# Cogito2012/OpenTAL

Hardware: AMD Instinct MI355X
Metric: clips/sec training step, 256-frame THUMOS14 clips (higher is better)
Workload: dtype bf16

## Files before the change

include/opental_hip.h:

```cpp
#ifndef OPENTAL_HIP_H
#define OPENTAL_HIP_H

#include <stdint.h>
#include <stddef.h>

#ifdef __cplusplus
extern "C" {
#endif

#define OTAL_ABI_VERSION 26

#define OTAL_E_NULL      (-1)
#define OTAL_E_SHAPE     (-2)
#define OTAL_E_ODD_C     (-3)
#define OTAL_E_BATCH     (-4)
#define OTAL_E_DTYPE     (-5)
#define OTAL_E_LEVELS    (-6)
#define OTAL_E_UNSUPPORTED (-7)

#define OTAL_F32  0
#define OTAL_BF16 1
#define OTAL_F16  2
#define OTAL_F64  3

#define OTAL_MAX_LEVELS 8

int otal_abi_version(void);
const char* otal_error_string(int code);
int otal_set_option(const char* name, int value);
int otal_get_option(const char* name, int dflt);
int otal_stream_wait(void* waiter, void* signaler);

int otal_bmp_fwd(const void* in, const float* seg, void* out,
                 int B, int C, int T, int N, int seg_batch, int dtype, void* stream);

int otal_bmp_bwd(const void* grad_out, const void* in, const float* seg, void* grad_in,
                 int B, int C, int T, int N, int seg_batch, int compat_ref_stride,
                 int dtype, void* stream);

int otal_bmp_fwd_levels(const void* in, const float* seg, void* out,
                        int B, int C, int nlev, const int* t_start, const int* n_start,
                        int dtype, void* stream);
int otal_bmp_bwd_levels(const void* grad_out, const void* in, const float* seg, void* grad_in,
                        int B, int C, int nlev, const int* t_start, const int* n_start,
                        int dtype, void* stream);

int otal_conv_half_storage(const int* geom, const int64_t* strides, int mode, int precision);
size_t otal_conv_workspace_bytes(const int* geom, int mode);

int otal_conv_fwd(const int* geom, const int64_t* strides, const float* x, const float* w,
                  const float* scale, const float* shift, float* y, int relu, int precision,
                  const void* prologue, void* ws, size_t ws_bytes, void* stream);

int otal_conv_dgrad(const int* geom, const int64_t* strides, const float* dy, const float* wt_packed,
                    float* dx, int accumulate, const float* out_mask, const float* out_scale,
                    int precision, const void* prologue, void* ws, size_t ws_bytes, void* stream);

int otal_conv_wgrad(const int* geom, const int64_t* strides, const float* x, const float* dy,
                    float* dw, int accumulate, int precision, const void* prologue, void* ws, size_t ws_bytes,
                    void* stream);

int otal_conv_fwd_pair(const int* geom, const int64_t* strides, const float* const* x, const float* const* w,
                       const float* const* scale, const float* const* shift, float* const* y, int relu, int precision,
                       const void* const* prologue, void* ws, size_t ws_bytes, void* stream);
int otal_conv_dgrad_pair(const int* geom, const int64_t* strides, const float* const* dy, const float* const* w,
                         float* const* dx, int precision, const void* const* prologue, void* ws, size_t ws_bytes, void* stream);
int otal_conv_wgrad_pair(const int* geom, const int64_t* strides, const float* const* x, const float* const* dy,
                         float* const* dw, int precision, void* ws, size_t ws_bytes, void* stream);

size_t otal_conv_prologue_bytes(const int* geom, const int64_t* strides, int mode, int precision);
size_t otal_conv_prologue_desc_bytes(void);
int otal_conv_prologue(const int* geom, const int64_t* strides, int mode, const float* w, int precision, void* region,
                       size_t region_bytes, void* host_desc, void* stream);
int otal_conv_prologue_batch(int n, const void* device_descs, const int* device_starts, int total_blocks, void* stream);

int otal_conv_defer_reduces(int on);
size_t otal_conv_deferred_end(void);
int otal_conv_deferred_count(void);
int otal_conv_flush_reduces(void* stream);

const char* otal_conv_last_kernel(void);

int otal_conv_pack_wt(const float* w, float* wt, int Cout, int Cin, int kvol, void* stream);

int otal_gn_relu_fwd(const float* x, const float* gamma, const float* beta, float* y, float* stats,
                     int B, int C, int T, int G, float eps, int relu, int nlev, const int* lev, void* stream);
int otal_gn_relu_bwd(const float* dy, int64_t dy_batch_stride, const float* x, const float* gamma, const float* beta,
                     const float* stats, float* dx, float* partial, int B, int C, int T, int G,
                     int relu, int nlev, const int* lev, void* stream);
int otal_gn_relu_fwd_pair(const float* const* x, const float* const* gamma, const float* const* beta, float* const* y,
                          float* const* stats, int B, int C, int T, int G, float eps, int relu, int nlev, const int* lev,
                          void* stream);
int otal_gn_relu_bwd_pair(const float* const* dy, const int64_t* dy_batch_stride, const float* const* x,
                          const float* const* gamma, const float* const* beta, const float* const* stats, float* const* dx,
                          float* const* partial, int B, int C, int T, int G, int relu, int nlev, const int* lev, void* stream);
int otal_sum_partials(int n_items, const float* const* partial, float* const* dst0, float* const* dst1,
                      float* const* dst2, const int* channels, const int* batches, void* stream);

const char* otal_layer_last_kernel(void);

int otal_maxpool3d_fwd(const int* geom, const int64_t* strides, const float* x, float* y,
                       unsigned char* argtap, void* stream);
int otal_maxpool3d_bwd(const int* geom, const int64_t* strides, const float* dy,
                       const unsigned char* argtap, float* dx, int accumulate,
                       const float* out_mask, const float* out_scale, void* stream);
size_t otal_maxpool3d_signbits_bytes(const int* geom, const int64_t* strides);
int otal_maxpool3d_fwd_signbits(const int* geom, const int64_t* strides, const float* x, float* y,
                                unsigned char* argtap, unsigned char* signbits, void* stream);
int otal_maxpool3d_bwd_signbits(const int* geom, const int64_t* strides, const float* dy, const unsigned char* argtap,
                                float* dx, int accumulate, const unsigned char* signbits, const float* out_scale,
                                void* stream);
int otal_maxpool3d_fwd_signbits_h(const int* geom, const int64_t* strides, const void* x_bf16, float* y,
                                  unsigned char* argtap, unsigned char* signbits, void* stream);
int otal_maxpool3d_bwd_signbits_h(const int* geom, const int64_t* strides, const float* dy, const unsigned char* argtap,
                                  void* dx_bf16, const unsigned char* signbits, const float* out_scale, void* stream);
int otal_maxpool3d_fwd_io(const int* geom, const int64_t* strides, const void* x, void* y, unsigned char* argtap,
                          unsigned char* signbits, int io, void* stream);
int otal_maxpool3d_bwd_io(const int* geom, const int64_t* strides, const void* dy, const unsigned char* argtap, void* dx,
                          int accumulate, const void* out_mask, const float* out_scale, const unsigned char* signbits, int io,
                          void* stream);
int otal_convert_storage(const void* src, int64_t src_bs, int64_t src_cs, void* dst, int64_t dst_bs, int64_t dst_cs,
                         int to_bf16, int B, int C, int P, void* stream);

int otal_head_outputs_fwd(int n_items, const int* channels, const int* modes, const float* const* raw, float* const* out,
                          float* const* unct, const float* scales, int B, int N, int nlev, const int* lev,
                          const float* level_strides, void* stream);
int otal_head_outputs_bwd(int n_items, const int* channels, const int* modes, const float* const* raw,
                          const float* const* out, const float* const* unct, const float* const* dout,
                          const float* const* dunct, float* const* draw, const float* scales, float* dscales, int B,
                          int N, int nlev, const int* lev, const float* level_strides, void* stream);

int otal_boundary_bce(const float* x, int64_t x_batch_stride, int64_t x_channel_stride, const float* mask,
                      int64_t mask_batch_stride, int64_t mask_row_stride, int mask_row0, int mask_step, float* terms,
                      float* dx, int B, int C, int T, void* stream);

int otal_boundary_finish(int n, const float* const* terms, const float* weights, const int* T, int B, float* out2, void* stream);
int otal_boundary_scale(int n, const float* const* dx, float* const* out, const float* weights, const int* C, const int* T,
                        int B, const float* g_start, const float* g_end, void* stream);

int otal_proposal_windows(const float* loc, float* seg, float* frame_seg, int B, int nlev,
                          const int* lev, float frame_num, void* stream);

int otal_decode_clips(const float* loc, const float* prop_loc, const float* priors, const float* conf,
                      const float* prop_conf, const float* center, const float* act, const float* prop_act,
                      const float* offsets, const float* fps, float* seg, float* score, float* unct,
                      float* actn, unsigned char* flag, int nclips, int A, int K, float clip_length,
                      float conf_thresh, void* stream);
int otal_decode_clips_ex(const float* loc, const float* prop_loc, const float* priors, const float* conf,
                         const float* prop_conf, const float* center, const float* act, const float* prop_act,
                         const float* offsets, const float* fps, float* seg, float* score, float* unct,
                         float* actn, unsigned char* flag, int nclips, int A, int K, float clip_length,
                         float conf_thresh, int score_fn, int first_class, void* stream);
int otal_decode_clips_ev(const float* loc, const float* prop_loc, const float* priors, const float* conf,
                         const float* prop_conf, const float* center, const float* act, const float* prop_act,
                         const float* offsets, const float* fps, float* seg, float* score, float* unct,
                         float* actn, unsigned char* flag, int nclips, int A, int K, float clip_length,
                         float conf_thresh, int score_fn, int first_class, int evidence, void* stream);
int otal_decode_clips_2s(const float* loc, const float* prop_loc, const float* conf, const float* prop_conf,
                         const float* center, const float* act, const float* prop_act, const float* flow_loc,
                         const float* flow_prop_loc, const float* flow_conf, const float* flow_prop_conf,
                         const float* flow_center, const float* flow_act, const float* flow_prop_act,
                         const float* unct_in, const float* prop_unct_in, const float* flow_unct_in,
                         const float* flow_prop_unct_in, const float* priors, const float* offsets, const float* fps,
                         float* seg, float* score, float* unct, float* actn, unsigned char* flag, int nclips, int A, int K,
                         float clip_length, float conf_thresh, int score_fn, int first_class, int evidence, int conf_sign,
                         void* stream);
int otal_softnms_classes(const float* seg, const float* score, const float* unct, const float* actn,
                         const unsigned char* flag, const int* clip_start, int nvideos, int max_clips,
                         int A, int K, float sigma, int top_k, float score_threshold, float* out,
                         int* counts, int* out_index, int out_cols, void* stream);
size_t otal_softnms_scratch_bytes(int total_clips, int max_clips, int A, int K);
int otal_softnms_classes_ws(const float* seg, const float* score, const float* unct, const float* actn,
                            const unsigned char* flag, const int* clip_start, int nvideos, int max_clips,
                            int A, int K, float sigma, int top_k, float score_threshold, float* out,
                            int* counts, int* out_index, int out_cols, void* scratch, size_t scratch_bytes,
                            int total_clips, void* stream);
int otal_detection_table(const float* rows, const int* counts, const double* durations, int V, int K, int top_k, int cols,
                         int drop_empty, int scoring, int* video, int* cls, double* seg, float* sup, double* known,
                         int* list_start, void* stream);
int otal_anchor_stats(const float* loc, const float* conf, const float* prop_conf, const float* center, const float* act,
                      const float* prop_act, const float* priors, const float* gt, const unsigned char* gvalid, int B, int K,
                      int C, int G, float clip_length, float overlap_thresh, int os_head, int n_known, int target,
                      int score_bins, int grad_bins, long long* hist_score, long long* hist_grad, int* label, float* value,
                      float* grad, void* stream);
int otal_anchor_stats_ev(const float* loc, const float* conf, const float* prop_conf, const float* center, const float* act,
                         const float* prop_act, const float* priors, const float* gt, const unsigned char* gvalid, int B,
                         int K, int C, int G, float clip_length, float overlap_thresh, int os_head, int n_known, int target,
                         int score_bins, int grad_bins, long long* hist_score, long long* hist_grad, int* label,
                         float* value, float* grad, int evidence, void* stream);

int otal_openmax_dist(const float* feat, int N, int rows_per_batch, int64_t sb, int64_t sr, int64_t sc, const float* mav,
                      int K, int D, const int* labels, float* dist, void* stream);
int otal_openmax_class_means(const float* feat, int N, int rows_per_batch, int64_t sb, int64_t sr, int64_t sc,
                             const int* labels, int K, int D, float* means, int* counts, void* stream);
int otal_openmax_probs(const float* logits, int64_t ldl, const float* feat, int N, int rows_per_batch, int64_t sb, int64_t sr,
                       int64_t sc, const float* mav, const float* wb, int K, int D, int R, float* probs, void* stream);
int otal_decode_clips_openmax(const float* loc, const float* prop_loc, const float* priors, const float* conf,
                              const float* prop_conf, const float* center, const float* offsets, const float* fps,
                              const float* feat, const float* prop_feat, const int64_t* feat_strides,
                              const int64_t* prop_feat_strides, const float* mav, const float* mav_prop, const float* wb,
                              const float* wb_prop, float* seg, float* score, float* unknown, unsigned char* flag,
                              int nclips, int A, int C, int first_class, int D, int R, int refined_feature,
                              float clip_length, float conf_thresh, void* stream);

int otal_openmax_dist_wide(const float* feat, int N, int rows_per_batch, int64_t sb, int64_t sr, int64_t sc, const float* mav,
                           int K, int D, const int* labels, float* dist, void* stream);
int otal_openmax_probs_wide(const float* logits, int64_t ldl, const float* feat, int N, int rows_per_batch, int64_t sb,
                            int64_t sr, int64_t sc, const float* mav, const float* wb, int K, int D, int R, float* probs,
                            void* stream);
int otal_decode_clips_openmax_wide(const float* loc, const float* prop_loc, const float* priors, const float* conf,
                                   const float* prop_conf, const float* center, const float* offsets, const float* fps,
                                   const float* feat, const float* prop_feat, const int64_t* feat_strides,
                                   const int64_t* prop_feat_strides, const float* mav, const float* mav_prop, const float* wb,
                                   const float* wb_prop, float* seg, float* score, float* unknown, unsigned char* flag,
                                   int nclips, int A, int C, int first_class, int D, int R, int refined_feature,
                                   float clip_length, float conf_thresh, void* stream);

int otal_head_convs_supported(int n_heads, int n_inputs, const int* in_idx, const int* cout, const int* ksize, int B, int C, int N);
int otal_head_convs_fwd(int n_heads, int n_inputs, const int* in_idx, const int* cout, const int* ksize,
                        const float* const* x, const float* const* w, const float* const* bias, float* const* y, int B, int C,
                        int N, int nlev, const int* lev, void* stream);
int otal_head_convs_bwd(int n_heads, int n_inputs, const int* in_idx, const int* cout, const int* ksize,
                        const float* const* x, const float* const* w, const float* const* dy, float* const* dx,
                        float* const* dw, float* const* db, int B, int C, int N, int nlev, const int* lev, void* stream);
int otal_head_convs_bwd_parts(int n_heads, int n_inputs, const int* in_idx, const int* cout, const int* ksize,
                        const float* const* x, const float* const* w, const float* const* dy, float* const* dx,
                        float* const* dw, float* const* db, int B, int C, int N, int nlev, const int* lev, int parts, void* stream);

int otal_rpl_head_fwd(const float* x, const float* centers, float* dist, int B, int C, int D, int N, void* stream);
int otal_rpl_head_bwd(const float* x, const float* centers, const float* g, float* dx, float* dcenters, int B, int C, int D,
                      int N, int parts, void* stream);

int otal_masked_scale_copy(const float* src, const int64_t* src_strides, const float* z, const int64_t* z_strides,
                           const float* scale, float* dst, const int64_t* dst_strides, int accumulate, int B, int C,
                           int T, int S, void* stream);

int otal_adam_flat(float* p, const float* g, float* m, float* v, int64_t n, float lr, float beta1,
                   float beta2, float eps, float weight_decay, int step, float grad_scale, void* stream);

int otal_adam_flat_dev(float* p, const float* g, float* m, float* v, int64_t n, float lr, float beta1,
                       float beta2, float eps, float weight_decay, const float* bias_corr, float grad_scale,
                       void* stream);

#define OTAL_GRAD_NORM_PARTIALS 2048
int otal_grad_norm(const float* g, int64_t n, float grad_scale, float max_norm, double* partials, float* out, void* stream);

int otal_adam_flat_clip(float* p, const float* g, float* m, float* v, int64_t n, float lr, float beta1, float beta2,
                        float eps, float weight_decay, const float* bias_corr, float grad_scale, const float* norm_coef,
                        void* stream);

size_t otal_detection_loss_scratch_floats(int B, int K);
size_t otal_detection_loss_grad_floats(int B, int K, int C);
int otal_detection_loss(const float* loc, const float* conf, const float* prop_loc, const float* prop_conf,
                        const float* center, const float* act, const float* prop_act, const float* priors,
                        const float* gt, const unsigned char* gvalid, float* weight_accum, int B, int K, int C, int G,
                        float clip_length, float overlap_thresh, int ibm_active, int num_bins, float momentum,
                        int iou_aware, int cls_mode, float focal_alpha, float* losses, float* grads, float* scratch,
                        void* stream);

int otal_detection_loss_ex(const float* loc, const float* conf, const float* prop_loc, const float* prop_conf,
                           const float* center, const float* act, const float* prop_act, const float* priors,
                           const float* gt, const unsigned char* gvalid, float* weight_accum, int B, int K, int C, int G,
                           float clip_length, float overlap_thresh, int ibm_active, int num_bins, float momentum,
                           int iou_aware, int cls_mode, float focal_alpha, int reweight, float rw_gamma, float* losses,
                           float* grads, float* scratch, void* stream);
int otal_detection_loss_ev(const float* loc, const float* conf, const float* prop_loc, const float* prop_conf,
                           const float* center, const float* act, const float* prop_act, const float* priors,
                           const float* gt, const unsigned char* gvalid, float* weight_accum, int B, int K, int C, int G,
                           float clip_length, float overlap_thresh, int ibm_active, int num_bins, float momentum,
                           int iou_aware, int cls_mode, float focal_alpha, int reweight, float rw_gamma, int evidence,
                           int loss_type, float* losses, float* grads, float* scratch, void* stream);

int otal_detection_loss_anet(const float* loc, const float* conf, const float* prop_loc, const float* prop_conf,
                             const float* center, const float* act, const float* prop_act, const float* priors2,
                             const float* gt, const unsigned char* gvalid, int B, int K, int C, int G,
                             float clip_length, float overlap_thresh, const float* level_bounds, int nlev,
                             int ibm_active, float ibm_coeff, int iou_aware, float act_weight, float act_margin,
                             float* losses, float* grads, float* scratch, void* stream);
int otal_detection_loss_anet_ex(const float* loc, const float* conf, const float* prop_loc, const float* prop_conf,
                                const float* center, const float* act, const float* prop_act, const float* priors2,
                                const float* gt, const unsigned char* gvalid, int B, int K, int C, int G,
                                float clip_length, float overlap_thresh, const float* level_bounds, int nlev,
                                int ibm_active, float ibm_coeff, int iou_aware, float act_weight, float act_margin,
                                int cls_mode, float focal_alpha, float* losses, float* grads, float* scratch, void* stream);
int otal_detection_loss_anet_ev(const float* loc, const float* conf, const float* prop_loc, const float* prop_conf,
                                const float* center, const float* act, const float* prop_act, const float* priors2,
                                const float* gt, const unsigned char* gvalid, int B, int K, int C, int G,
                                float clip_length, float overlap_thresh, const float* level_bounds, int nlev,
                                int ibm_active, float ibm_coeff, int iou_aware, float act_weight, float act_margin,
                                int cls_mode, float focal_alpha, int evidence, int loss_type, float* losses, float* grads,
                                float* scratch, void* stream);

int otal_detection_loss_rpl(const float* loc, const float* conf, const float* prop_loc, const float* prop_conf,
                            const float* center, const float* priors, const float* gt, const unsigned char* gvalid,
                            int B, int K, int C, int G, float clip_length, float overlap_thresh, int gcpl,
                            float temperature, float weight_pl, float radius, float* losses, float* grads, float* scratch,
                            void* stream);

int otal_detection_loss_bwd(const float* grads, const float* const* g7, float* out, int B, int K, int C, void* stream);

int otal_prepare_clips(const unsigned char* frames, const void* params, float* out, int B, int T, int Hs, int Ws,
                       int Ho, int Wo, void* stream);
int otal_prepare_clips_map(const unsigned char* frames, const void* params, const int* frame_map, float* out,
                           float* out_ssl, int B, int T, int Hs, int Ws, int Ho, int Wo, void* stream);
int otal_prepare_clips_ch(const unsigned char* frames, const void* params, const int* frame_map, float* out, float* out_ssl,
                          int B, int C_src, int C_out, int T, int Hs, int Ws, int Ho, int Wo, void* stream);

int otal_prepare_windows(const void* params, float* out, int B, int C, int T, int H, int W, void* stream);


int otal_pyramid_merge_fwd(const float* p0, const float* p1, float* packed, float* frame, int B, int C, int t0, int T,
                           int up, void* stream);
int otal_pyramid_merge_bwd(const float* da, const float* db, const float* dframe, const float* dnext, float* dp0, float* dp1,
                           int B, int C, int t0, int T, int up, void* stream);
int otal_gn_relu_fwd_to(const float* x, const float* gamma, const float* beta, float* y, int64_t y_bs, int64_t y_cs,
                        float* stats, int B, int C, int T, int G, float eps, int relu, int nlev, const int* lev, void* stream);
int otal_gn_relu_fwd_pair_to(const float* const* x, const float* const* gamma, const float* const* beta, float* const* y,
                             int64_t y_bs, int64_t y_cs, float* const* stats, int B, int C, int T, int G, float eps, int relu,
                             int nlev, const int* lev, void* stream);

int otal_gn_relu_bwd_sum(int n_terms, const float* const* dy, const int64_t* dy_bs, const int64_t* dy_cs, const int* dy_T,
                         const float* x, const float* gamma, const float* beta, const float* stats, float* dx, float* partial,
                         int B, int C, int T, int G, int relu, int nlev, const int* lev, void* stream);

int otal_bmp_fwd_levels_to(const float* in, const float* seg, float* out, int64_t pooled_bs, int B, int C, int nlev,
                           const int* t_start, const int* n_start, void* stream);
int otal_bmp_bwd_levels_from(const float* grad_out, int64_t pooled_bs, const float* in, const float* seg, float* grad_in, int B,
                             int C, int nlev, const int* t_start, const int* n_start, void* stream);

#define OTAL_EVAL_MAX_GT 1024
int otal_eval_match(const double* pred_seg, const int* pred_start, const double* gt_seg, const int* gt_start,
                    const double* thresholds, int ngroups, int nthr, int* out, int* nonfinite, void* stream);

int otal_eval_match_labeled(const double* pred_seg, const int* pred_label, const int* pred_start, const double* gt_seg,
                            const int* gt_label, const int* gt_start, const double* thresholds, int ngroups, int nthr, int* out,
                            double* max_tiou, int* nonfinite, void* stream);

#define OTAL_AP_TILE 256
#define OTAL_AP_MAX_CLASS_ROWS (2147483647 - OTAL_AP_TILE)
int otal_average_precision(const int* codes, const int* rank_pos, const int* class_start, const int* gt_count, int N, int K,
                           int nthr, double* ap, void* stream);

int otal_open_set_curves(const double* known, const int* flags, int M, int nthr, double* out, void* stream);

#define OTAL_WI_MAX_GT 16777216
int otal_wilderness_impact(const int* codes, const int* pred_label, const int* gt_label, int n_known, int n_unknown, int N,
                           int M, int nthr, int K, double* out, void* stream);

#ifdef __cplusplus
}
#endif
#endif
```

opental_amd/common/i3d_backbone.py:

```python
import torch
import torch.nn as nn
import torch.nn.functional as F
from torch.autograd import Function

from . import ops
from .layers import MaxPool3dSamePadding

ONE, THREE = (1, 1, 1), (3, 3, 3)
BN_EPS = 1e-3


class Unit3D(nn.Module):

    def __init__(self, in_channels, output_channels, kernel_shape=(1, 1, 1), stride=(1, 1, 1), padding=0,
                 activation_fn=F.relu, use_batch_norm=True, use_bias=False, padding_valid_spatial=False,
                 name='unit_3d'):
        super(Unit3D, self).__init__()
        if not use_batch_norm or use_bias or activation_fn is not F.relu or padding_valid_spatial or padding == -1:
            raise NotImplementedError("backbone Unit3D is conv(no bias) + BN + ReLU with SAME padding")
        self._output_channels = output_channels
        self._kernel_shape = tuple(kernel_shape)
        self._stride = tuple(stride)
        self.name = name
        self.conv3d = nn.Conv3d(in_channels, output_channels, self._kernel_shape, self._stride, padding=0, bias=False)
# ... 6 lines not shown

    def forward(self, x):
        scale, shift = self.folded_bn()
        return I3DFeaturesFunction.apply(x, [("conv", 0, self._kernel_shape, self._stride)], ("out",), scale, shift,
                                         [0, scale.numel()], self.conv3d.weight)[0]


class InceptionModule(nn.Module):
    def __init__(self, in_channels, out_channels, name):
        super(InceptionModule, self).__init__()
        oc = out_channels
        self.b0 = Unit3D(in_channels, oc[0], ONE, name=name + '/Branch_0/Conv3d_0a_1x1')
        self.b1a = Unit3D(in_channels, oc[1], ONE, name=name + '/Branch_1/Conv3d_0a_1x1')
        self.b1b = Unit3D(oc[1], oc[2], THREE, name=name + '/Branch_1/Conv3d_0b_3x3')
        self.b2a = Unit3D(in_channels, oc[3], ONE, name=name + '/Branch_2/Conv3d_0a_1x1')
        self.b2b = Unit3D(oc[3], oc[4], THREE, name=name + '/Branch_2/Conv3d_0b_3x3')
        self.b3a = MaxPool3dSamePadding(kernel_size=[3, 3, 3], stride=(1, 1, 1), padding=0)
        self.b3b = Unit3D(in_channels, oc[5], ONE, name=name + '/Branch_3/Conv3d_0b_1x1')
        self.name = name
        self.out_channels = tuple(oc)

    def units(self):
        return [self.b0, self.b1a, self.b1b, self.b2a, self.b2b, self.b3b]

    def fused_1x1_weights(self):
        return [self.b1a.conv3d.weight, self.b2a.conv3d.weight, self.b0.conv3d.weight]


_ENDPOINTS = (
    ('Conv3d_1a_7x7', 'conv', (None, 64, (7, 7, 7), (2, 2, 2))),
    ('MaxPool3d_2a_3x3', 'pool', ((1, 3, 3), (1, 2, 2))),
    ('Conv3d_2b_1x1', 'conv', (64, 64, ONE, ONE)),
    ('Conv3d_2c_3x3', 'conv', (64, 192, THREE, ONE)),
    ('MaxPool3d_3a_3x3', 'pool', ((1, 3, 3), (1, 2, 2))),
    ('Mixed_3b', 'mixed', (192, (64, 96, 128, 16, 32, 32))),
    ('Mixed_3c', 'mixed', (256, (128, 128, 192, 32, 96, 64))),
    ('MaxPool3d_4a_3x3', 'pool', (THREE, (2, 2, 2))),
    ('Mixed_4b', 'mixed', (480, (192, 96, 208, 16, 48, 64))),
    ('Mixed_4c', 'mixed', (512, (160, 112, 224, 24, 64, 64))),
    ('Mixed_4d', 'mixed', (512, (128, 128, 256, 24, 64, 64))),
    ('Mixed_4e', 'mixed', (512, (112, 144, 288, 32, 64, 64))),
    ('Mixed_4f', 'mixed', (528, (256, 160, 320, 32, 128, 128))),
    ('MaxPool3d_5a_2x2', 'pool', ((2, 2, 2), (2, 2, 2))),
    ('Mixed_5b', 'mixed', (832, (256, 160, 320, 32, 128, 128))),
    ('Mixed_5c', 'mixed', (832, (384, 192, 384, 48, 128, 128))),
)


class ExtendWeightFunction(Function):

    @staticmethod
    def forward(ctx, w2, buf):
        if w2.dim() != 5 or w2.shape[1] != 2 or tuple(buf.shape) != (w2.shape[0], 3) + tuple(w2.shape[2:]) \
                or buf.dtype != w2.dtype or buf.device != w2.device:
            raise RuntimeError("ExtendWeightFunction: a (Cout,2,kt,kh,kw) weight and a (Cout,3,kt,kh,kw) buffer of its dtype / device")
        buf[:, :2].copy_(w2.detach())
        ctx.w2 = w2
        return buf.detach()

    @staticmethod
    def backward(ctx, g3):
        w2, ctx.w2 = ctx.w2, None
        slot = ops.grad_slot(w2) if g3.is_cuda else None
        if slot is not None:
            slot.copy_(g3[:, :2])
            return slot, None
        return g3[:, :2].contiguous(), None


def check_clip_planes(weight_channels, x):
    from .input_pipeline import is_zero_plane
    planes = int(x.shape[1])
    if weight_channels == 2 and planes == 3:
        if not is_zero_plane(x):
            raise RuntimeError("a 2-channel (optical-flow) network was handed a 3-plane clip batch that is not flagged as a "
                               "zero-plane flow batch (rgb frames?): flow batches come from ClipStager(channels=2) / "
                               "prepare_clips on (T,H,W,2) frames")
        return True
    if is_zero_plane(x) and weight_channels != 2:
        raise RuntimeError(f"a zero-plane optical-flow batch was handed to a network with {weight_channels} input channels "
                           "(in_channels must be 2)")
    if planes != weight_channels:
        raise RuntimeError(f"clip batch has {planes} planes, the network's first layer takes {weight_channels} "
                           "(rgb clips have 3, optical-flow clips 2)")
    return False


class InceptionI3d(nn.Module):
    VALID_ENDPOINTS = tuple(n for n, _, _ in _ENDPOINTS) + ('Logits', 'Predictions')

    def __init__(self, num_classes=400, spatial_squeeze=True, final_endpoint='Mixed_5c', name='inception_i3d',
                 in_channels=3, dropout_keep_prob=0.5):
        super(InceptionI3d, self).__init__()
        if final_endpoint not in self.VALID_ENDPOINTS:
            raise ValueError('Unknown final endpoint %s' % final_endpoint)
        if final_endpoint in ('Logits', 'Predictions'):
            raise NotImplementedError("the detection path stops at Mixed_5c (BDNet.py:27)")
        self._final_endpoint = final_endpoint
        self.end_points = {}
        for ep, kind, args in _ENDPOINTS:
            if kind == 'conv':
                cin, cout, k, s = args
                self.end_points[ep] = Unit3D(in_channels if cin is None else cin, cout, k, s, name=name + ep)
            elif kind == 'pool':
                self.end_points[ep] = MaxPool3dSamePadding(kernel_size=list(args[0]), stride=args[1], padding=0)
            else:
                self.end_points[ep] = InceptionModule(args[0], list(args[1]), name + ep)
            if ep == final_endpoint:
                break
        self._plan = None

    def build(self):
        for k in self.end_points.keys():
            self.add_module(k, self.end_points[k])

    def _make_plan(self):
        plan, units = [], []
        for ep, kind, args in _ENDPOINTS:
            if ep not in self.end_points:
                break
            mod = self.end_points[ep]
            if kind == 'conv':
                plan.append(("conv", len(units), mod._kernel_shape, mod._stride))
                units.append(mod)
            elif kind == 'pool':
                plan.append(("pool", tuple(mod.kernel_size), tuple(mod.stride)))
            else:
                plan.append(("mixed", len(units), mod.out_channels))
                units += mod.units()
            plan[-1] = plan[-1] + (ep,)
        return plan, units

    def extract_features(self, x, endpoints=('Mixed_4f', 'Mixed_5c')):
        if self._plan is None:
            self._plan = self._make_plan()
        plan, units = self._plan
        zero_plane = check_clip_planes(int(units[0].conv3d.weight.shape[1]), x)
        for u in units:
            if u.bn.training or (torch.is_grad_enabled() and u.bn.weight.requires_grad):
                raise NotImplementedError("I3D BatchNorm must be frozen (freeze_bn + freeze_bn_affine, BDNet.py:39-49)")
        key = tuple((u.bn.weight._version, u.bn.bias._version, u.bn.running_mean._version, u.bn.running_var._version,
                     u.bn.weight.data_ptr(), u.bn.running_var.data_ptr()) for u in units)
        if getattr(self, "_fold_key", None) != key:
            folded = [u.folded_bn() for u in units]
            offs = [0]
            for sc, _ in folded:
                offs.append(offs[-1] + sc.numel())
            self._fold = (torch.cat([sc for sc, _ in folded]), torch.cat([sh for _, sh in folded]), offs)
            self._fold_key = key
        scale, shift, offs = self._fold
        weights = [u.conv3d.weight for u in units]
        if zero_plane:
            weights[0] = ExtendWeightFunction.apply(weights[0], self._extended_weight(weights[0]))
        cut = self._stem_cut(plan, endpoints) if self.split_backward else 0
        if cut:
            (stem_out,) = I3DFeaturesFunction.apply(x, plan[:cut], ("=" + plan[cut - 1][-1],), scale, shift, offs, *weights)
            self.stem_out = cut_in = stem_out
            if self.detach_cut and torch.is_grad_enabled() and stem_out.requires_grad:
                self.cut_leaf = cut_in = stem_out.detach().requires_grad_(True)
            outs = I3DFeaturesFunction.apply(cut_in, plan[cut:], tuple(endpoints), scale, shift, offs, *weights)
        else:
            self.stem_out = None
            outs = I3DFeaturesFunction.apply(x, plan, tuple(endpoints), scale, shift, offs, *weights)
        return dict(zip(endpoints, outs))

    _w3 = None

    def _extended_weight(self, w2):
        buf = self._w3
        if buf is None or buf.device != w2.device or buf.dtype != w2.dtype:
            if w2.is_cuda and torch.cuda.is_current_stream_capturing():
                raise RuntimeError("the zero-plane weight buffer cannot be created inside a graph capture: run one eager "
                                   "forward pass of the flow network first")
            buf = self._w3 = torch.zeros((w2.shape[0], 3) + tuple(w2.shape[2:]), dtype=w2.dtype, device=w2.device)
        return buf

    split_backward = False
    detach_cut = False
    stem_out = None
    cut_leaf = None
    STEM_CUT_AFTER = 'MaxPool3d_4a_3x3'

    def _stem_cut(self, plan, endpoints):
        names = [st[-1] for st in plan]
        if self.STEM_CUT_AFTER not in names:
            return 0
        cut = names.index(self.STEM_CUT_AFTER) + 1
        if cut >= len(plan) or any(e in names[:cut] for e in endpoints):
            return 0
        return cut

    def stem_parameters(self):
        if self._plan is None:
            self._plan = self._make_plan()
        plan, units = self._plan
        cut = self._stem_cut(plan, ())
        idx = set()
        for st in plan[:cut]:
            if st[0] == "conv":
                idx.add(st[1])
            elif st[0] == "mixed":
                idx.update(range(st[1], st[1] + 6))
        return [units[i].conv3d.weight for i in sorted(idx)]

    def forward(self, x):
        raise NotImplementedError("classification logits are not part of the detection path; use extract_features")


_FUSED_AFFINE = {}


def _fused_weight(w_b1a, w_b2a, w_b0):
    n1, n2 = w_b1a.numel(), w_b2a.numel()
    es = w_b1a.element_size()
    if (w_b1a.is_contiguous() and w_b2a.is_contiguous() and w_b0.is_contiguous()
            and w_b2a.data_ptr() == w_b1a.data_ptr() + n1 * es and w_b0.data_ptr() == w_b2a.data_ptr() + n2 * es
            and w_b1a.untyped_storage().data_ptr() == w_b0.untyped_storage().data_ptr()):
        rows = w_b1a.shape[0] + w_b2a.shape[0] + w_b0.shape[0]
        return w_b1a.as_strided((rows,) + tuple(w_b1a.shape[1:]), w_b1a.stride(), w_b1a.storage_offset())
    return torch.cat([w_b1a, w_b2a, w_b0], 0)


def _cat_cached(cache, owner, tag, parts):
    key = (owner.data_ptr(), owner._version, tag)
    hit = cache.get(key)
    if hit is None:
        hit = (torch.cat(parts), owner)
        if len(cache) > 256:
            cache.clear()
        cache[key] = hit
    return hit[0]


_OUT_SCALE = {}


def _fused_affine(scale, shift, offs, w0):
    key = (scale.data_ptr(), shift.data_ptr(), scale._version, w0)
    hit = _FUSED_AFFINE.get(key)
    if hit is None:
        pick = lambda t, i: t[offs[i]:offs[i + 1]]
        hit = (torch.cat([pick(scale, w0 + 1), pick(scale, w0 + 3), pick(scale, w0)]),
               torch.cat([pick(shift, w0 + 1), pick(shift, w0 + 3), pick(shift, w0)]), scale, shift)
        if len(_FUSED_AFFINE) > 256:
            _FUSED_AFFINE.clear()
        _FUSED_AFFINE[key] = hit
    return hit[0], hit[1]


_HALF_OK = {}


def _pool_half_ok(shape, k, s):
    _, _, T, H, W = shape
    k, s = tuple(k), tuple(s)
    out_positions = -(-T // s[0]) * -(-H // s[1]) * -(-W // s[2])
    if out_positions % 8:
        return False
    if k[1:] == (3, 3) and s[1:] == (2, 2) and H % 2 == 0 and W % 4 == 0:
        return (k[0], s[0]) == (1, 1) or ((k[0], s[0]) == (3, 2) and T % 2 == 0)
    return k == THREE and s == ONE and H == W and H in (12, 6)


def _conv_half_ok(shape, cout, k, first=False):
    modes = (0, 2) if first else (0, 1, 2)
    return all(ops.half_storage_ok(m, tuple(shape), cout, k, ONE, both=True) for m in modes)


def _step_half_ok(step, shape, weights):
    key = (step[0], tuple(shape), step[1:-1] if step[0] != "conv" else (tuple(weights[step[1]].shape), step[2], step[3]), ops.HALF_CHAIN,
           int(ops.CONV_PRECISION), ops.HALF_STORAGE)
    hit = _HALF_OK.get(key)
    if hit is None:
        B, C, T, H, W = shape
        if not (ops.HALF_CHAIN and ops.HALF_STORAGE and int(ops.CONV_PRECISION) & 1):
            hit = False
        elif step[0] == "conv":
            hit = tuple(step[3]) == ONE and _conv_half_ok(shape, weights[step[1]].shape[0], tuple(step[2]))
        elif step[0] == "pool":
            hit = _pool_half_ok(shape, step[1], step[2])
        else:
            oc = step[2]
            hit = (_conv_half_ok(shape, oc[1] + oc[3] + oc[0], ONE) and _conv_half_ok((B, oc[1], T, H, W), oc[2], THREE)
                   and _conv_half_ok((B, oc[3], T, H, W), oc[4], THREE) and _pool_half_ok(shape, THREE, ONE)
                   and _conv_half_ok(shape, oc[5], ONE))
        if len(_HALF_OK) > 512:
            _HALF_OK.clear()
        _HALF_OK[key] = hit
    return hit


class I3DFeaturesFunction(Function):

    @staticmethod
    def forward(ctx, x, plan, endpoints, scale, shift, offs, *weights):
        x = x.contiguous()
        sc = lambda i: scale[offs[i]:offs[i + 1]]
        sh = lambda i: shift[offs[i]:offs[i + 1]]
        tape, found, half_grads = [], {}, {}
        cur = x
        cur_scale = None
        BF = torch.bfloat16
        need_grad = any(ctx.needs_input_grad)
        raw_out = {e[1:] for e in endpoints if e.startswith("=")}
        endpoints = tuple(e.lstrip("=") for e in endpoints)

        def leave_half():
            nonlocal cur
            cur32 = ops.convert_storage(cur, torch.float32)
            tape.append(("cvt", cur, cur32, cur_scale))
            cur = cur32

        for si, step in enumerate(plan):
            kind, name = step[0], step[-1]
            chain = cur.dtype == BF and _step_half_ok(step, cur.shape, weights)
            pool_io1 = (cur.dtype == BF and not chain and kind == "pool" and cur_scale is not None
                        and tuple(step[1]) == (1, 3, 3) and tuple(step[2]) == (1, 2, 2)
                        and cur.shape[3] % 2 == 0 and cur.shape[4] % 4 == 0)
            if cur.dtype == BF and not chain and not pool_io1:
                leave_half()
            if kind == "conv" and chain:
                _, wi, k, s, _ = step
                y = ops.conv_forward(cur, weights[wi], k, s, scale=sc(wi), shift=sh(wi), relu=True)
                tape.append(("conv", wi, k, s, cur, y, cur_scale, sc(wi)))
                cur, cur_scale = y, sc(wi)
            elif kind == "conv":
                _, wi, k, s, _ = step
                pooled_next = (name not in endpoints and si + 1 < len(plan) and plan[si + 1][0] == "pool"
                               and tuple(plan[si + 1][1]) == (1, 3, 3) and tuple(plan[si + 1][2]) == (1, 2, 2)
                               and ops.half_storage_ok(0, tuple(cur.shape), weights[wi].shape[0], k, s))
                grad_half = (pooled_next and si == 0 and not x.requires_grad
                             and ops.half_storage_ok(2, tuple(cur.shape), weights[wi].shape[0], k, s))
                half = pooled_next and (grad_half or (si > 0 and ops.HALF_ACT_DIRECT))
                if (not half and si == 0 and not x.requires_grad and ops.HALF_CHAIN and si + 1 < len(plan) and name not in endpoints
                        and ops.half_storage_ok(0, tuple(cur.shape), weights[wi].shape[0], k, s)
                        and ops.half_storage_ok(2, tuple(cur.shape), weights[wi].shape[0], k, s)):
                    half = True
                half_grads[si + 1] = grad_half
                y = ops.conv_forward(cur, weights[wi], k, s, scale=sc(wi), shift=sh(wi), relu=True, half_out=half)
                tape.append(("conv", wi, k, s, cur, y, cur_scale, sc(wi)))
                cur, cur_scale = y, sc(wi)
            elif kind == "pool":
                _, k, s, _ = step
                if chain:
                    y, arg, bits = ops.maxpool3d_forward(cur, k, s, signbits=True, half_out=True)
                elif cur_scale is not None:
                    y, arg, bits = ops.maxpool3d_forward(cur, k, s, signbits=True)
                else:
                    (y, arg), bits = ops.maxpool3d_forward(cur, k, s), None
                tape.append(("pool", k, s, cur, (arg, bits, half_grads.get(si, False)), cur_scale, None))
                cur, cur_scale = y, None
            else:
                _, w0, oc, _ = step
                B, _, T, H, W = cur.shape
                ctot = oc[0] + oc[2] + oc[4] + oc[5]
                o1, o13 = oc[1], oc[1] + oc[3]
                Z = torch.empty((B, o13 + ctot, T, H, W), dtype=cur.dtype, device=cur.device)
                h1, h2, Y = Z[:, :o1], Z[:, o1:o13], Z[:, o13:]
                c1, c2, c3 = oc[0], oc[0] + oc[2], oc[0] + oc[2] + oc[4]
                wf = _fused_weight(weights[w0 + 1].detach(), weights[w0 + 3].detach(), weights[w0].detach())
                scf, shf = _fused_affine(scale, shift, offs, w0)
                ops.conv_forward(cur, wf, ONE, ONE, scale=scf, shift=shf, relu=True, out=Z[:, :o13 + c1])
                lane = ops.branch_lane(cur.device)
                if lane.on:
                    lane.fork()
                    with lane:
                        ops.conv_forward(h2, weights[w0 + 4], THREE, ONE, scale=sc(w0 + 4), shift=sh(w0 + 4), relu=True,
                                         out=Y[:, c2:c3])
                        pm, argm = ops.maxpool3d_forward(cur, THREE, ONE, half_out=chain)
                        ops.conv_forward(pm, weights[w0 + 5], ONE, ONE, scale=sc(w0 + 5), shift=sh(w0 + 5), relu=True,
                                         out=Y[:, c3:])
                    ops.conv_forward(h1, weights[w0 + 2], THREE, ONE, scale=sc(w0 + 2), shift=sh(w0 + 2), relu=True,
                                     out=Y[:, c1:c2])
                    lane.join()
                else:
                    ops.conv_forward(h1, weights[w0 + 2], THREE, ONE, scale=sc(w0 + 2), shift=sh(w0 + 2), relu=True,
                                     out=Y[:, c1:c2])
                    ops.conv_forward(h2, weights[w0 + 4], THREE, ONE, scale=sc(w0 + 4), shift=sh(w0 + 4), relu=True,
                                     out=Y[:, c2:c3])
                    pm, argm = ops.maxpool3d_forward(cur, THREE, ONE, half_out=chain)
                    ops.conv_forward(pm, weights[w0 + 5], ONE, ONE, scale=sc(w0 + 5), shift=sh(w0 + 5), relu=True,
                                     out=Y[:, c3:])
                out_scale = _cat_cached(_OUT_SCALE, scale, w0, [sc(w0), sc(w0 + 2), sc(w0 + 4), sc(w0 + 5)])
                tape.append(("mixed", w0, (c1, c2, c3), cur, h1, h2, pm, argm, Y, cur_scale, (wf, o1, o13), out_scale))
                cur, cur_scale = Y, out_scale
            if name in endpoints:
                if cur.dtype == BF and name not in raw_out:
                    ends = si + 1 == len(plan) or not _step_half_ok(plan[si + 1], cur.shape, weights)
                    if need_grad or ends:
                        leave_half()
                        found[name] = (cur, len(tape))
                    else:
                        found[name] = (ops.convert_storage(cur, torch.float32), len(tape))
                else:
                    found[name] = (cur, len(tape))
                hooks = ops.STEP.endpoint_hooks
                hook = hooks.get(name) if hooks else None
                if hook is not None:
                    hook(found[name][0])
        missing = [e for e in endpoints if e not in found]
        if missing:
            raise RuntimeError(f"unknown endpoints {missing}")
        ctx.tape = tape
        ctx.meta = (scale, offs, [found[e][1] for e in endpoints], len(weights), x.requires_grad)
        ctx.weights = weights
        ctx.outs = [found[e][0] for e in endpoints]
        return tuple(ctx.outs)

    @staticmethod
    def backward(ctx, *douts):
        tape, weights = ctx.tape, ctx.weights
        scale, offs, out_pos, nw, need_dx = ctx.meta
        sc = lambda i: scale[offs[i]:offs[i + 1]]
        dws = [None] * nw
        pending = {}
        for pos, g, z in zip(out_pos, douts, ctx.outs):
            if g is not None:
                pending.setdefault(pos, []).append((g, z, tape[pos - 1][-1]))
        zg = {}

        def out_grad_buffer(p, shape, like):
            if p >= 1 and tape[p - 1][0] == "mixed":
                o13 = tape[p - 1][10][2]
                B, ct, T, H, W = shape
                buf = torch.empty((B, o13 + ct, T, H, W), dtype=like.dtype, device=like.device)
                zg[p] = buf
                return buf[:, o13:]
            return torch.empty(tuple(shape), dtype=like.dtype, device=like.device)

        side = ops.side_wgrads(weights[0].device)
        in_slots = True
        dcur = None
        cloned = True
        mixed_pos = [p for p in range(1, len(tape) + 1) if tape[p - 1][0] == "mixed"]
        tail_below = min(mixed_pos) if mixed_pos and not need_dx else 0
        for pos in range(len(tape), 0, -1):
            if pos == tail_below - 1 and not any(pending.get(q) for q in range(1, pos + 1)):
                ops.late_mark([weights[st[1]] for st in tape[:pos] if st[0] == "conv"])
            for g, z, zs in pending.pop(pos, ()):
                ops.join_pending(g)
                dense = g.dim() == 5 and (g.shape[4] == 1 or g.stride(4) == 1) and (g.shape[3] == 1 or g.stride(3) == g.shape[4])
                if zs is not None and not dense:
                    g = g.contiguous()
                if dcur is None:
                    if zs is not None:
                        dcur = out_grad_buffer(pos, g.shape, g)
                        ops.masked_scale_copy(g, z, zs, dcur)
                    elif tape[pos - 1][0] == "mixed":
                        dcur = out_grad_buffer(pos, g.shape, g)
                        dcur.copy_(g)
                    else:
                        dcur = g.contiguous()
                        cloned = False
                elif zs is not None:
                    ops.masked_scale_copy(g, z, zs, dcur, accumulate=True)
                else:
                    if not cloned:
                        dcur, cloned = dcur.clone(), True
                    dcur.add_(g)
            if dcur is None:
                continue
            step = tape[pos - 1]
            first = pos == 1
            if step[0] == "cvt":
                _, xh, _, _ = step
                dcur = ops.convert_storage(dcur.contiguous(), xh.dtype, out=out_grad_buffer(pos - 1, xh.shape, xh))
            elif step[0] == "conv":
                _, wi, k, s, xin, y, in_scale, _ = step
                slot = ops.grad_slot(weights[wi])
                in_slots = in_slots and slot is not None
                if first and not need_dx:
                    side.issue()
                    dws[wi] = ops.conv_wgrad(xin, dcur, weights[wi].shape, k, s, out=slot)
                else:
                    dws[wi] = side.wgrad(xin, dcur, weights[wi].shape, k, s, out=slot)
                if first and not need_dx:
                    dcur = None
                else:
                    dcur = ops.conv_dgrad(dcur, weights[wi], xin.shape, k, s, out=out_grad_buffer(pos - 1, xin.shape, xin),
                                          out_mask=xin if in_scale is not None else None, out_scale=in_scale)
                side.flush()
                ops.grads_ready([(weights[wi], dws[wi])])
            elif step[0] == "pool":
                _, k, s, xin, (arg, bits, grad_half), in_scale, _ = step
                if dcur.dtype == torch.bfloat16:
                    masked = in_scale is not None and bits is not None
                    dcur = ops.maxpool3d_backward(dcur, arg, xin.shape, k, s, out=out_grad_buffer(pos - 1, xin.shape, xin),
                                                  out_scale=in_scale if masked else None, out_signbits=bits if masked else None)
                elif grad_half:
                    dcur = ops.maxpool3d_backward(dcur, arg, xin.shape, k, s, out_scale=in_scale, out_signbits=bits, half_out=True)
                else:
                    dcur = ops.maxpool3d_backward(dcur, arg, xin.shape, k, s, out=out_grad_buffer(pos - 1, xin.shape, dcur),
                                                  out_mask=xin if (in_scale is not None and bits is None) else None,
                                                  out_scale=in_scale, out_signbits=bits)
            else:
                _, w0, (c1, c2, c3), xin, h1, h2, pm, argm, Y, in_scale, (wf, o1, o13), _ = step
                Zg = zg.pop(pos)
                dY = Zg[:, o13:]
                dX = out_grad_buffer(pos - 1, xin.shape, xin)
                xm = xin if in_scale is not None else None
                sl = (slice(0, c1), slice(c1, c2), slice(c2, c3), slice(c3, Y.shape[1]))
                for a, b, hid, sli, dst in ((w0 + 1, w0 + 2, h1, sl[1], Zg[:, :o1]), (w0 + 3, w0 + 4, h2, sl[2], Zg[:, o1:o13])):
                    g = dY[:, sli]
                    slot = ops.grad_slot(weights[b])
                    in_slots = in_slots and slot is not None
                    dws[b] = side.wgrad(hid, g, weights[b].shape, THREE, ONE, out=slot)
                    ops.conv_dgrad(g, weights[b], hid.shape, THREE, ONE, out=dst, out_mask=hid, out_scale=sc(a))
                gf = Zg[:, :o13 + c1]
                slot = ops.grad_slot(wf)
                in_slots = in_slots and slot is not None
                dwf = side.wgrad(xin, gf, wf.shape, ONE, ONE, out=slot)
                dws[w0 + 1], dws[w0 + 3], dws[w0] = dwf[:o1], dwf[o1:o13], dwf[o13:]
                ops.conv_dgrad(gf, wf, xin.shape, ONE, ONE, out=dX, out_mask=xm, out_scale=in_scale)
                g3 = dY[:, sl[3]]
                slot = ops.grad_slot(weights[w0 + 5])
                in_slots = in_slots and slot is not None
                dws[w0 + 5] = side.wgrad(pm, g3, weights[w0 + 5].shape, ONE, ONE, out=slot)
                dpm = ops.conv_dgrad(g3, weights[w0 + 5], pm.shape, ONE, ONE)
                ops.maxpool3d_backward(dpm, argm, xin.shape, THREE, ONE, out=dX, accumulate=True,
                                       out_mask=xm, out_scale=in_scale)
                dcur = dX
                side.flush()
                ops.grads_ready([(weights[w0 + q], dws[w0 + q]) for q in range(6)])
        side.node_end(in_slots)
        ctx.tape = None
        ctx.outs = None
        dx = dcur if need_dx else None
        return (dx, None, None, None, None, None) + tuple(dws)
```

opental_amd/common/ops.py:

```python
import bisect
import ctypes
import os
import warnings
from typing import NamedTuple

import torch

from .. import _lib as L
from .conv_geom import make_geom

_WORKSPACE = {}
WORKSPACE_BYTES = 192 << 20
WORKSPACE_TOTAL = 512 << 20

CONV_PROFILE = None

CONV_PRECISION = 0
HALF_STORAGE = os.environ.get("OTAL_HALF_STORAGE", "1") != "0"
HALF_ACT_DIRECT = os.environ.get("OTAL_HALF_ACT_DIRECT", "0") != "0"
HALF_CHAIN = os.environ.get("OTAL_HALF_CHAIN", "1") != "0"


def _prof_begin():
    if CONV_PROFILE is None:
# ... 322 lines not shown
        return on.__exit__(*exc)


def branch_lane(device):
    key = (device.type, device.index)
    b = _BRANCHES.get(key)
    if b is None:
        b = _BRANCHES[key] = BranchLane(device)
    return b


_EARLY = {}


def early_lane(device):
    key = (device.type, device.index)
    b = _EARLY.get(key)
    if b is None:
        b = _EARLY[key] = BranchLane(device, ws_index=3)
    return b


def join_pending(t):
    joins = STEP.pending_joins
    lane = joins.pop(t.data_ptr(), None) if joins else None
    if lane is not None:
        lane.join()


_CAPTURE_STREAMS = {}


def capture_stream(device):
    key = (device.type, device.index)
    st = _CAPTURE_STREAMS.get(key)
    if st is None:
        st = _CAPTURE_STREAMS[key] = torch.cuda.Stream(device=device)
    return st


def side_wgrads(device):
    key = (device.type, device.index)
    sd = _SIDES.get(key)
    if sd is None:
        sd = _SIDES[key] = SideWgrads(device)
    return sd


def late_mark(weights):
    s = STEP
    if s.lanes is None or s.late_weights is not None:
        return
    side_issue()
    s.lanes.cut(("mark",))
    s.late_weights = list(weights)


def take_late_weights():
    w, STEP.late_weights = STEP.late_weights, None
    return w


def side_join():
    for sd in _SIDES.values():
        sd.join()


def side_issue():
    for sd in _SIDES.values():
        sd.issue()


def side_busy():
    return any(sd.keep for sd in _SIDES.values())


def _as5(t):
    if t.dim() == 3:
        return t.unsqueeze(-1).unsqueeze(-1)
    if t.dim() != 5:
        raise RuntimeError("expected a (B,C,T) or (B,C,T,H,W) tensor")
    return t


def _check(t5, name, dtype=torch.float32):
    if not t5.is_cuda:
        raise RuntimeError(f"{name}: opental_amd ops run on the GPU only (no CPU fallback)")
    if t5.dtype != dtype:
        raise RuntimeError(f"{name}: {dtype} expected, got {t5.dtype}")
    _, _, T, H, W = t5.shape
    exp = {4: 1, 3: W, 2: H * W}
    for d, e in exp.items():
        if t5.shape[d] > 1 and t5.stride(d) != e:
            raise RuntimeError(f"{name}: spatial dims must be dense (stride {t5.stride()})")
    if t5.shape[1] > 1 and t5.stride(1) < T * H * W:
        raise RuntimeError(f"{name}: bad channel stride")


def _bs(t5):
    _, C, T, H, W = t5.shape
    cs = t5.stride(1) if C > 1 else T * H * W
    bs = t5.stride(0) if t5.shape[0] > 1 else cs * C
    return bs, cs


_GEOM_CACHE = {}


def _geom_arrays(g, x5, y5):
    xb, xc = _bs(x5)
    yb, yc = _bs(y5)
    key = (tuple(g), xb, xc, yb, yc)
    hit = _GEOM_CACHE.get(key)
    if hit is None:
        hit = ((ctypes.c_int * len(g))(*g), (ctypes.c_int64 * 4)(xb, xc, yb, yc))
        _GEOM_CACHE[key] = hit
    return hit


_MAKE_GEOM_CACHE = {}


def _make_geom(B, Cin, Cout, in_thw, k, s, levels, spatial_valid):
    if levels is not None and tuple(k) == (1, 1, 1) and tuple(s) == (1, 1, 1):
        levels = None
    key = (B, Cin, Cout, tuple(in_thw), k, s, levels if levels is None else tuple(levels), spatial_valid)
    hit = _MAKE_GEOM_CACHE.get(key)
    if hit is None:
        hit = make_geom(B, Cin, Cout, in_thw, k, s, levels, spatial_valid)
        _MAKE_GEOM_CACHE[key] = hit
    return hit


def _opt(t):
    return L.ptr(t) if t is not None else None


def _k3(k):
    return (k, 1, 1) if isinstance(k, int) else tuple(k)



class PrologueCache:

    def __init__(self, persistent_range=None):
        self.persistent_range = persistent_range
        self.entries = {}
        self.descs = []
        self.blocks = []
        self.dev_starts = None
        self.dev_descs = None
        self.dirty = False

    def region(self, mode, ga, sa, key, w, prec):
        if key in self.entries:
            return self.entries[key]
        lib = L.lib()
        nbytes = lib.otal_conv_prologue_bytes(ga, sa, mode, prec)
        if nbytes == 0:
            self.entries[key] = None
            return None
        dev = w.device if w is not None else torch.device("cuda", torch.cuda.current_device())
        reg = torch.empty(nbytes, dtype=torch.uint8, device=dev)
        desc = ctypes.create_string_buffer(lib.otal_conv_prologue_desc_bytes())
        rc = lib.otal_conv_prologue(ga, sa, mode, _opt(w), prec, L.ptr(reg), nbytes, desc, L.stream())
        if rc < 0:
            raise RuntimeError(f"otal_conv_prologue failed: {rc}")
        if rc > 0:
            self.descs.append(desc.raw)
            self.blocks.append(int(rc))
            self.dirty = True
        self.entries[key] = reg
        return reg

    def refresh(self):
        if not self.descs:
            return
        if self.dirty:
            host = torch.frombuffer(bytearray(b"".join(self.descs)), dtype=torch.uint8)
            dev = next(iter(v for v in self.entries.values() if v is not None)).device
            self.dev_descs = host.to(dev)
            starts = [0]
            for nb in self.blocks:
                starts.append(starts[-1] + nb)
            self.dev_starts = torch.tensor(starts, dtype=torch.int32).to(dev)
            self.total_blocks = starts[-1]
            self.dirty = False
        L.check(L.lib().otal_conv_prologue_batch(len(self.descs), L.ptr(self.dev_descs), L.ptr(self.dev_starts),
                                                 self.total_blocks, L.stream()), "otal_conv_prologue_batch")


def activate_prologues(cache):
    STEP.prologues = cache
    if cache is not None:
        cache.refresh()


def deactivate_prologues():
    STEP.prologues = None


def _prologue(mode, ga, sa, pkey, w, prec):
    c = STEP.prologues
    if c is None or not (prec & 1):
        return None
    wp = 0
    if mode != 2:
        wp = w.data_ptr()
        r = c.persistent_range
        if r is None or not (r[0] <= wp < r[1]):
            return None
    reg = c.region(mode, ga, sa, (wp, pkey, prec), w, prec)
    if reg is None:
        return None
    return L.ptr(reg)


_PLANS = {}


def _plan(mode, xs, ys, Cout, k, s, levels, spatial_valid, xname, yname):
    key = (mode, xs.shape, xs.stride(), ys.shape, ys.stride(), Cout, k, s, levels, spatial_valid, xs.dtype, ys.dtype,
           xs.device, ys.device)
    plan = _PLANS.get(key)
    if plan is None:
        x5, y5 = _as5(xs), _as5(ys)
        B, Cin, Ti, Hi, Wi = x5.shape
        g, outn = _make_geom(B, Cin, Cout, (Ti, Hi, Wi), k, s, levels, spatial_valid)
        if tuple(y5.shape) != (B, Cout) + outn:
            raise RuntimeError(f"{yname} has shape {tuple(y5.shape)}, expected {(B, Cout) + outn}")
        _check(x5, xname, x5.dtype)
        _check(y5, yname, y5.dtype)
        ga, sa = _geom_arrays(g, x5, y5)
        plan = (g, ga, sa, (mode, tuple(g), _bs(x5), _bs(y5)), (tuple(x5.shape), _bs(x5)))
        if len(_PLANS) > 4096:
            _PLANS.clear()
        _PLANS[key] = plan
    return plan


def _out_positions(x, Cout, k, s, levels, spatial_valid):
    x5 = _as5(x)
    B, Cin, Ti, Hi, Wi = x5.shape
    return _make_geom(B, Cin, Cout, (Ti, Hi, Wi), k, s, levels, spatial_valid)[1]


def half_storage_ok(mode, x_shape, cout, k, s, both=False):
    if not (HALF_STORAGE and int(CONV_PRECISION) & 1) or len(x_shape) != 5:
        return False
    k, s = _k3(k), _k3(s)
    B, Cin, Ti, Hi, Wi = x_shape
    g, outn = _make_geom(B, Cin, cout, (Ti, Hi, Wi), k, s, None, False)
    ga = (ctypes.c_int * len(g))(*g)
    P = outn[0] * outn[1] * outn[2]
    sa = (ctypes.c_int64 * 4)(Cin * Ti * Hi * Wi, Ti * Hi * Wi, cout * P, P)
    return bool(L.lib().otal_conv_half_storage(ga, sa, int(mode), int(CONV_PRECISION) | (12 if both else 0)))


def conv_forward(x, w, k, s, scale=None, shift=None, relu=False, spatial_valid=False, levels=None, out=None, half_out=False):
    k, s = _k3(k), _k3(s)
    if levels is not None:
        levels = tuple(levels)
    Cout = w.shape[0]
    if x.dtype == torch.bfloat16:
        return _conv_forward_half(x, w, k, s, scale, shift, relu, spatial_valid, levels, out)
    if out is None:
        outn = _out_positions(x, Cout, k, s, levels, spatial_valid)
        out = torch.empty((x.shape[0], Cout) + (outn if x.dim() == 5 else outn[:1]),
                          dtype=torch.bfloat16 if half_out else x.dtype, device=x.device)
    if out.dtype != (torch.bfloat16 if half_out else torch.float32) or x.dtype != torch.float32:
        raise RuntimeError("conv_forward: float32 tensors (bfloat16 y with half_out)")
    g, ga, sa, pkey, _ = _plan(0, x, out, Cout, k, s, levels, spatial_valid, "x", "y")
    if not w.is_contiguous():
        raise RuntimeError("weights must be contiguous")
    wsp, wsn = _ws_args(x.device)
    ev = _prof_begin()
    prec = int(CONV_PRECISION)
    pre = _prologue(0, ga, sa, pkey, w, prec)
    L.check(L.lib().otal_conv_fwd(ga, sa, L.ptr(x), L.ptr(w), _opt(scale), _opt(shift), L.ptr(out), int(relu),
                                  prec | (4 if half_out else 0), pre, wsp, wsn, L.stream()),
            "otal_conv_fwd")
    _prof_end(ev, "fwd", g)
    return out


def _conv_forward_half(x, w, k, s, scale, shift, relu, spatial_valid, levels, out):
    Cout = w.shape[0]
    if out is None:
        outn = _out_positions(x, Cout, k, s, levels, spatial_valid)
        out = torch.empty((x.shape[0], Cout) + (outn if x.dim() == 5 else outn[:1]), dtype=torch.bfloat16, device=x.device)
    if out.dtype != torch.bfloat16 or not (int(CONV_PRECISION) & 1):
        raise RuntimeError("conv_forward: a bfloat16 x needs a bfloat16 y and the bf16-operand mode")
    g, ga, sa, pkey, _ = _plan(0, x, out, Cout, k, s, levels, spatial_valid, "x", "y")
    if not w.is_contiguous():
        raise RuntimeError("weights must be contiguous")
    wsp, wsn = _ws_args(x.device)
    ev = _prof_begin()
    prec = int(CONV_PRECISION)
    pre = _prologue(0, ga, sa, pkey, w, prec)
    L.check(L.lib().otal_conv_fwd(ga, sa, L.ptr(x), L.ptr(w), _opt(scale), _opt(shift), L.ptr(out), int(relu),
                                  prec | 12, pre, wsp, wsn, L.stream()), "otal_conv_fwd (bf16 tensors)")
    _prof_end(ev, "fwd", g)
    return out


def pack_wt(w):
    Cout, Cin = w.shape[0], w.shape[1]
    kvol = w[0, 0].numel()
    wt = torch.empty((Cin, Cout, kvol), dtype=w.dtype, device=w.device)
    L.check(L.lib().otal_conv_pack_wt(L.ptr(w), L.ptr(wt), Cout, Cin, kvol, L.stream()), "otal_conv_pack_wt")
    return wt


def conv_dgrad(dy, w, x_shape, k, s, spatial_valid=False, levels=None, out=None,
               accumulate=False, wt=None, out_mask=None, out_scale=None):
    k, s = _k3(k), _k3(s)
    if levels is not None:
        levels = tuple(levels)
    Cout = w.shape[0]
    if out is None:
        if accumulate:
            raise RuntimeError("accumulate needs an existing buffer")
        out = torch.empty(tuple(x_shape), dtype=dy.dtype, device=dy.device)
    elif tuple(out.shape) != tuple(x_shape):
        raise RuntimeError(f"conv_dgrad: out has shape {tuple(out.shape)}, expected {tuple(x_shape)}")
    half = dy.dtype == torch.bfloat16
    if out.dtype != dy.dtype or not (half or dy.dtype == torch.float32):
        raise RuntimeError("conv_dgrad: float32 tensors, or bfloat16 dy / dx / out_mask together")
    if half and (accumulate or not (int(CONV_PRECISION) & 1)):
        raise RuntimeError("conv_dgrad: bfloat16 tensors need the bf16-operand mode and a plain store")
    g, ga, sa, pkey, xlay = _plan(1, out, dy, Cout, k, s, levels, spatial_valid, "dx", "dy")
    prec = int(CONV_PRECISION)
    if wt is None:
        wt = w if w.is_contiguous() else w.contiguous()
        prec |= 2
    wsp, wsn = _ws_args(dy.device)
    ev = _prof_begin()
    if out_mask is not None:
        m5 = _as5(out_mask)
        if (tuple(m5.shape), _bs(m5)) != xlay or out_mask.dtype != dy.dtype:
            raise RuntimeError("out_mask must share dx's shape, layout and dtype")
    pre = _prologue(1, ga, sa, pkey, wt, prec) if (prec & 2) else None
    if half:
        prec |= 12 | (16 if out_mask is not None else 0)
    L.check(L.lib().otal_conv_dgrad(ga, sa, L.ptr(dy), L.ptr(wt), L.ptr(out),
                                    int(accumulate), _opt(out_mask), _opt(out_scale), prec, pre,
                                    wsp, wsn, L.stream()),
            "otal_conv_dgrad")
    _prof_end(ev, "dgrad", g)
    return out


def is_full_collapse(x_shape, k, s, spatial_valid):
    return (spatial_valid and len(x_shape) == 5 and tuple(x_shape[3:]) == tuple(k[1:]) and k[0] == 1
            and tuple(s) == (1, 1, 1))


def conv_dgrad_collapse(dy, w, x_shape):
    B, Cin, T, H, W = x_shape
    Cout = w.shape[0]
    wa = w.detach().reshape(1, Cout, Cin * H * W)
    dyt = dy.reshape(B, Cout, T).permute(0, 2, 1).reshape(B * T, Cout, 1).contiguous()
    dxp = conv_forward(wa, dyt, 1, 1)
    return dxp.view(B, T, Cin, H, W).permute(0, 2, 1, 3, 4)


def masked_scale_copy(src, z, scale, dst, accumulate=False):
    B, C, T, H, W = dst.shape
    S = H * W
    for name, t in (("src", src), ("z", z), ("dst", dst)):
        if not t.is_cuda or t.dtype != torch.float32 or tuple(t.shape) != (B, C, T, H, W):
            raise RuntimeError(f"masked_scale_copy: {name} must be a float32 GPU tensor of shape {(B, C, T, H, W)}")
        if (W > 1 and t.stride(4) != 1) or (H > 1 and t.stride(3) != W):
            raise RuntimeError(f"masked_scale_copy: {name} needs dense H x W planes (strides {t.stride()})")
    st = lambda t: (ctypes.c_int64 * 3)(t.stride(0), t.stride(1), t.stride(2))
    L.check(L.lib().otal_masked_scale_copy(L.ptr(src), st(src), L.ptr(z), st(z), _opt(scale), L.ptr(dst), st(dst),
                                           int(accumulate), B, C, T, S, L.stream()), "otal_masked_scale_copy")
    return dst


class GradSlots:

    def __init__(self, flat, grad, offsets, numels):
        self.base, self.n, self.grad = flat.data_ptr(), flat.numel(), grad
        self.offsets, self.numels = list(offsets), list(numels)
        self.written = [False] * len(self.offsets)

    def reset(self):
        self.written = [False] * len(self.offsets)

    def take(self, w):
        if w.dtype != torch.float32 or not w.is_contiguous():
            return None
        off = w.data_ptr() - self.base
        if off < 0 or off % 4 or off // 4 + w.numel() > self.n:
            return None
        off //= 4
        i = bisect.bisect_left(self.offsets, off)
        if i == len(self.offsets) or self.offsets[i] != off:
            return None
        j, cur, end = i, off, off + w.numel()
        while j < len(self.offsets) and cur < end:
            cur += self.numels[j]
            j += 1
        if cur != end:
            return None
        if any(self.written[i:j]):
            flush_pending_sums()
            flush_reduces()
            return None
        for q in range(i, j):
            self.written[q] = True
        return self.grad[off:end].view(w.shape)

    def release(self, w):
        off = (w.data_ptr() - self.base) // 4
        i = bisect.bisect_left(self.offsets, off)
        j, cur, end = i, off, off + w.numel()
        while j < len(self.offsets) and cur < end:
            self.written[j] = False
            cur += self.numels[j]
            j += 1


def grads_ready(pairs):
    flush_reduces()
    cb = STEP.ready
    if cb is not None:
        cb(pairs)


def grad_slot(w):
    slots = STEP.slots
    return slots.take(w) if slots is not None and "OTAL_NO_GRAD_SLOTS" not in os.environ else None


def conv_wgrad(x, dy, w_shape, k, s, spatial_valid=False, levels=None, out=None, accumulate=False):
    k, s = _k3(k), _k3(s)
    if levels is not None:
        levels = tuple(levels)
    Cout = w_shape[0]
    half_dy = dy.dtype == torch.bfloat16
    half_x = x.dtype == torch.bfloat16
    if not (half_x or x.dtype == torch.float32) or not (half_dy or dy.dtype == torch.float32) or (half_x and not half_dy):
        raise RuntimeError("conv_wgrad: float32 x with a float32 or bfloat16 dy, or both bfloat16")
    g, ga, sa, pkey, _ = _plan(2, x, dy, Cout, k, s, levels, spatial_valid, "x", "dy")
    if out is None:
        if accumulate:
            raise RuntimeError("accumulate needs an existing buffer")
        out = torch.empty(tuple(w_shape), dtype=torch.float32, device=x.device)
    if not out.is_contiguous():
        raise RuntimeError("dw must be contiguous")
    st = STEP
    if st.defer and (accumulate or (st.defer_owner is not None and st.defer_owner[0] != st.ws_index)):
        flush_reduces()
    wsp, wsn = _ws_args(x.device)
    ev = _prof_begin()
    prec = int(CONV_PRECISION)
    pre = _prologue(2, ga, sa, pkey, x, prec) if (half_x or not half_dy) else None
    L.check(L.lib().otal_conv_wgrad(ga, sa, L.ptr(x), L.ptr(dy), L.ptr(out),
                                    int(accumulate), prec | (4 if half_dy else 0) | (8 if half_x else 0), pre, wsp, wsn, L.stream()),
            "otal_conv_wgrad")
    if st.defer:
        _after_wgrad(x.device)
    _prof_end(ev, "wgrad", g)
    return out


PAIR_LAUNCHES = os.environ.get("OTAL_PAIR_LAUNCHES", "1") != "0"
_VP2 = ctypes.c_void_p * 2


def _pp(a, b):
    return _VP2(a.data_ptr() if a is not None else None, b.data_ptr() if b is not None else None)


def _same_layout(a, b):
    return a.shape == b.shape and a.stride() == b.stride() and a.dtype == b.dtype and a.device == b.device


def conv_forward_pair(xs, ws, k, s, shifts=None, levels=None):
    k, s = _k3(k), _k3(s)
    if levels is not None:
        levels = tuple(levels)
    if not PAIR_LAUNCHES or not (int(CONV_PRECISION) & 1) or not _same_layout(xs[0], xs[1]) or ws[0].shape != ws[1].shape:
        return None
    if xs[0].dtype != torch.float32 or not (ws[0].is_contiguous() and ws[1].is_contiguous()):
        return None
    Cout = ws[0].shape[0]
    outn = _out_positions(xs[0], Cout, k, s, levels, False)
    ys = [torch.empty((x.shape[0], Cout) + outn[:1], dtype=x.dtype, device=x.device) for x in xs]
    g, ga, sa, pkey, _ = _plan(0, xs[0], ys[0], Cout, k, s, levels, False, "x", "y")
    prec = int(CONV_PRECISION)
    pres = [_prologue(0, ga, sa, pkey, w, prec) for w in ws]
    if (pres[0] is None) != (pres[1] is None):
        return None
    wsp, wsn = _ws_args(xs[0].device)
    ev = _prof_begin()
    sh = None if shifts is None or shifts[0] is None else _pp(shifts[0], shifts[1])
    rc = L.lib().otal_conv_fwd_pair(ga, sa, _pp(*xs), _pp(*ws), None, sh, _pp(*ys), 0, prec,
                                    None if pres[0] is None else _VP2(pres[0].value, pres[1].value), wsp, wsn, L.stream())
    if rc == L.E_UNSUPPORTED:
        return None
    L.check(rc, "otal_conv_fwd_pair")
    _prof_end(ev, "fwd", g, 2)
    return ys


def conv_dgrad_pair(dys, ws, x_shape, k, s, levels=None):
    k, s = _k3(k), _k3(s)
    if levels is not None:
        levels = tuple(levels)
    if not PAIR_LAUNCHES or not (int(CONV_PRECISION) & 1) or not _same_layout(dys[0], dys[1]) or ws[0].shape != ws[1].shape:
        return None
    if dys[0].dtype != torch.float32 or not (ws[0].is_contiguous() and ws[1].is_contiguous()):
        return None
    Cout = ws[0].shape[0]
    outs = [torch.empty(tuple(x_shape), dtype=dy.dtype, device=dy.device) for dy in dys]
    g, ga, sa, pkey, _ = _plan(1, outs[0], dys[0], Cout, k, s, levels, False, "dx", "dy")
    prec = int(CONV_PRECISION) | 2
    pres = [_prologue(1, ga, sa, pkey, w, prec) for w in ws]
    if (pres[0] is None) != (pres[1] is None):
        return None
    wsp, wsn = _ws_args(dys[0].device)
    ev = _prof_begin()
    rc = L.lib().otal_conv_dgrad_pair(ga, sa, _pp(*dys), _pp(*ws), _pp(*outs), prec,
                                      None if pres[0] is None else _VP2(pres[0].value, pres[1].value), wsp, wsn, L.stream())
    if rc == L.E_UNSUPPORTED:
        return None
    L.check(rc, "otal_conv_dgrad_pair")
    _prof_end(ev, "dgrad", g, 2)
    return outs


def conv_wgrad_pair(xs, dys, w_shape, k, s, levels=None, outs=(None, None)):
    k, s = _k3(k), _k3(s)
    if levels is not None:
        levels = tuple(levels)
    if not PAIR_LAUNCHES or not (int(CONV_PRECISION) & 1) or not _same_layout(xs[0], xs[1]) or not _same_layout(dys[0], dys[1]):
        return None
    if xs[0].dtype != torch.float32 or dys[0].dtype != torch.float32:
        return None
    Cout = w_shape[0]
    g, ga, sa, pkey, _ = _plan(2, xs[0], dys[0], Cout, k, s, levels, False, "x", "dy")
    outs = [o if o is not None else torch.empty(tuple(w_shape), dtype=torch.float32, device=xs[0].device) for o in outs]
    if not (outs[0].is_contiguous() and outs[1].is_contiguous()):
        return None
    st = STEP
    if st.defer and st.defer_owner is not None and st.defer_owner[0] != st.ws_index:
        flush_reduces()
    wsp, wsn = _ws_args(xs[0].device)
    ev = _prof_begin()
    rc = L.lib().otal_conv_wgrad_pair(ga, sa, _pp(*xs), _pp(*dys), _pp(*outs), int(CONV_PRECISION), wsp, wsn, L.stream())
    if rc == L.E_UNSUPPORTED:
        return None
    L.check(rc, "otal_conv_wgrad_pair")
    if st.defer:
        _after_wgrad(xs[0].device)
    _prof_end(ev, "wgrad", g, 2)
    return outs


def gn_relu_forward_pair(xs, gammas, betas, groups=32, eps=1e-5, relu=True, levels=None, outs=None):
    if not PAIR_LAUNCHES or not _same_layout(xs[0], xs[1]) or not xs[0].is_contiguous():
        return None
    L.require_device(*xs, *gammas, *betas)
    B, C, T = xs[0].shape
    nlev, lev = _lev_arg(levels)
    stats = [torch.empty((B, groups, nlev, 2), dtype=torch.float32, device=x.device) for x in xs]
    if outs is not None:
        st0, st1 = _dest_strides(outs[0], B, C, T), _dest_strides(outs[1], B, C, T)
        if st0 != st1:
            return None
        rc = L.lib().otal_gn_relu_fwd_pair_to(_pp(*xs), _pp(*gammas), _pp(*betas), _pp(*outs), st0[0], st0[1], _pp(*stats),
                                              B, C, T, groups, eps, int(relu), nlev, lev, L.stream())
        if rc == L.E_UNSUPPORTED:
            return None
        L.check(rc, "otal_gn_relu_fwd_pair_to")
        return list(zip(outs, stats))
    ys = [torch.empty_like(x) for x in xs]
    rc = L.lib().otal_gn_relu_fwd_pair(_pp(*xs), _pp(*gammas), _pp(*betas), _pp(*ys), _pp(*stats), B, C, T, groups,
                                       eps, int(relu), nlev, lev, L.stream())
    if rc == L.E_UNSUPPORTED:
        return None
    L.check(rc, "otal_gn_relu_fwd_pair")
    return list(zip(ys, stats))


def _lev_arg(levels):
    if levels is None or len(levels) <= 2:
        return 1, None
    return len(levels) - 1, L.int_array(list(levels))


def _dest_strides(out, B, C, T):
    if tuple(out.shape) != (B, C, T) or out.dtype != torch.float32 or not out.is_cuda or (T > 1 and out.stride(2) != 1):
        raise RuntimeError("gn_relu_forward: `out` must be a float32 (B,C,T) GPU tensor with dense positions")
    cs = out.stride(1) if C > 1 else T
    return (out.stride(0) if B > 1 else cs * C), cs


def gn_relu_forward(x, gamma, beta, groups=32, eps=1e-5, relu=True, levels=None, out=None):
    L.require_device(x, gamma, beta)
    B, C, T = x.shape
    nlev, lev = _lev_arg(levels)
    stats = torch.empty((B, groups, nlev, 2), dtype=torch.float32, device=x.device)
# ... 909 lines not shown
```

opental_amd/csrc/conv1a_tile.h:

```cpp
#pragma once
#include <hip/hip_runtime.h>
#include <stdint.h>

namespace otal_conv {

struct Conv1aTileArgs {
    const float* x;
    const float* w;
    const unsigned short* wp;
    void* out;
    const float* scale;
    const float* shift;
    int64_t x_bs, x_cs, y_bs, y_cs;
    int B, Ti, Hi, To, Ho, M;
    int relu, half;
    int flags;
};

__attribute__((visibility("hidden"))) int launch_conv1a_tile(const Conv1aTileArgs& a, void* ws, size_t ws_bytes, hipStream_t st);

}
```

opental_amd/csrc/conv1a_tile.hip:

```cpp
#include "common.h"
#include "conv1a_tile.h"
#include "conv_select.h"
#include <type_traits>

namespace {

typedef float f32x16 __attribute__((ext_vector_type(16)));
typedef short bf16x8 __attribute__((ext_vector_type(8)));
struct Words4 { unsigned a, b, c, d; };
struct Words2 { unsigned a, b; };
typedef float f32x4 __attribute__((ext_vector_type(4)));
typedef unsigned u32x4 __attribute__((ext_vector_type(4)));
typedef __bf16 hw_bf16x2 __attribute__((ext_vector_type(2)));
typedef float hw_f32x2 __attribute__((ext_vector_type(2)));
__device__ __forceinline__ unsigned cvt_pk_bf16(float lo, float hi) {
    const hw_f32x2 f = {lo, hi};
    return __builtin_bit_cast(unsigned, __builtin_convertvector(f, hw_bf16x2));
}

template <int I, int N, class F>
__device__ __forceinline__ void static_for(F&& f) {
    if constexpr (I < N) {
        f(std::integral_constant<int, I>{});
        static_for<I + 1, N>(f);
    }
}

constexpr int TT = C1T_TT, TR = C1T_TR, WO = 48;
constexpr int NPL = 2 * TT + 5, NR = 2 * TR + 5;
constexpr int NC = 102, PITCH = NC * 8, PLANE = NR * PITCH;
constexpr int NT = 512, NWAVE = NT / 64, WPOS = TT * TR * WO / NWAVE;
constexpr int BM = 64, WM = 2, WN = WPOS / 32;
constexpr int STEPS = 49;
constexpr int EPI_PITCH = WPOS * 2 + 16;
constexpr int QPR = 24, IPP = NR * QPR;
static_assert(TT * TR * WO == NWAVE * WPOS && WPOS % 32 == 0 && (TR * WO) % WPOS == 0, "a wave's positions lie in one output plane");
static_assert(NPL * PLANE + 2 * BM * 4 <= 160 * 1024 && NWAVE * BM * EPI_PITCH <= NPL * PLANE, "LDS");

struct TileAt {
    int b, to0, ho0, mblk;
};

__global__ __launch_bounds__(NT) void conv1a_tile_fwd_kernel(const otal_conv::Conv1aTileArgs a, int nwork, int per_wg, int tm) {
    __shared__ __attribute__((aligned(16))) unsigned char patch[NPL * PLANE];
    __shared__ __attribute__((aligned(16))) float rows[2 * BM];
    const int tid = threadIdx.x, lane = tid & 63;
    const int wave = __builtin_amdgcn_readfirstlane(tid >> 6);
    const int tiles_h = a.Ho / TR, tiles_t = a.To / TT;
    int wg = blockIdx.x;
    if ((gridDim.x & 7) == 0) wg = (wg & 7) * (gridDim.x >> 3) + (wg >> 3);
    const int w_begin = wg * per_wg, w_end = min(nwork, w_begin + per_wg);
    if (w_begin >= w_end) return;
    auto tile_at = [&](int w) {
        TileAt t;
        t.mblk = w % tm; w /= tm;
        const int th = w % tiles_h; w /= tiles_h;
        t.to0 = (w % tiles_t) * TT;
        t.b = w / tiles_t;
        t.ho0 = th * TR;
        return t;
    };
    const unsigned cs_bytes = (unsigned)(a.x_cs * 4);
    const int x_extent = (int)((2 * a.x_cs + (int64_t)a.Ti * a.Hi * 96) * 4);

    auto item_issue = [&](const TileAt& t, int e, int pl0, int plstep, int nitems, f32x4 (&v)[3], int& off) {
        const auto rx = __builtin_amdgcn_make_buffer_rsrc(const_cast<float*>(a.x + (int64_t)t.b * a.x_bs), 0, x_extent, 0x00020000);
        const bool live = e < nitems;
        const int gi = e / IPP, rem = e - gi * IPP, rr = rem / QPR, q = rem - rr * QPR;
        const int pl = pl0 + plstep * gi;
        const int ti = 2 * t.to0 - 2 + pl, hi = 2 * t.ho0 - 2 + rr;
        const bool ok = live && (unsigned)ti < (unsigned)a.Ti && (unsigned)hi < (unsigned)a.Hi;
        const bool ld = ok;
        off = live ? pl * PLANE + rr * PITCH + (4 * q + 2) * 8 : -1;
        const unsigned vo = ld ? (unsigned)((((int64_t)ti * a.Hi + hi) * 96 + 4 * q) * 4) : 0xffffffffu;
#pragma unroll
        for (int ci = 0; ci < 3; ++ci)
            v[ci] = __builtin_bit_cast(f32x4, __builtin_amdgcn_raw_buffer_load_b128(rx, vo, ci * cs_bytes, 0));
    };
    auto item_commit = [&](const f32x4 (&v)[3], int off) {
        if (off < 0) return;
        u32x4 lo, hi;
        lo[0] = cvt_pk_bf16(v[0][0], v[1][0]); lo[1] = cvt_pk_bf16(v[2][0], 0.f);
        lo[2] = cvt_pk_bf16(v[0][1], v[1][1]); lo[3] = cvt_pk_bf16(v[2][1], 0.f);
        hi[0] = cvt_pk_bf16(v[0][2], v[1][2]); hi[1] = cvt_pk_bf16(v[2][2], 0.f);
        hi[2] = cvt_pk_bf16(v[0][3], v[1][3]); hi[3] = cvt_pk_bf16(v[2][3], 0.f);
        *reinterpret_cast<u32x4*>(patch + off) = lo;
        *reinterpret_cast<u32x4*>(patch + off + 16) = hi;
    };

    const auto rw = __builtin_amdgcn_make_buffer_rsrc(const_cast<unsigned short*>(a.wp), 0, (int)((int64_t)tm * BM * STEPS * 64), 0x00020000);
    constexpr int WD = 2;

    const int lt = wave >> 1;
    int xbase[WN];
#pragma unroll
    for (int j = 0; j < WN; ++j) {
        const int o = (wave & 1) * WPOS + j * 32 + (lane & 31);
        const int lr = o / WO, wo = o - lr * WO;
        xbase[j] = ((2 * lt) * NR + 2 * lr) * PITCH + (2 * wo) * 8 + (lane >> 5) * 16;
    }

    f32x4 pv[3][3];
    int poff[3];
    TileAt cur = tile_at(w_begin);
#pragma unroll
    for (int u = 0; u < 3; ++u) item_issue(cur, tid + NT * u, 0, 2, 4 * IPP, pv[u], poff[u]);

    auto begin_tile = [&](const TileAt& t, int tid_l) {
        if (tid_l < BM) {
            const int m = t.mblk * BM + tid_l;
            rows[2 * tid_l] = (m < a.M && a.scale) ? a.scale[m] : 1.f;
            rows[2 * tid_l + 1] = (m < a.M && a.shift) ? a.shift[m] : 0.f;
        }
        for (int i = tid_l; i < NPL * NR * 6; i += NT) {
            const int row = i / 6, e = i - row * 6;
            *reinterpret_cast<Words2*>(patch + row * PITCH + (e < 2 ? e : 96 + e) * 8) = Words2{0u, 0u};
        }
#pragma unroll
        for (int u = 0; u < 3; ++u) item_commit(pv[u], poff[u]);
    };
    begin_tile(cur, tid);

    for (int work = w_begin; work < w_end; ++work) {
        const int m0 = cur.mblk * BM;
        int tid_l = tid;
        asm volatile("" : "+v"(tid_l));
        const int lane_l = tid_l & 63;
        const unsigned wvo = (unsigned)(cur.mblk * (BM * STEPS * 64) + lane * 16);
        bf16x8 aw[WD][2][WM];
        auto load_w = [&](int s) {
#pragma unroll
            for (int kk = 0; kk < 2; ++kk)
#pragma unroll
                for (int i = 0; i < WM; ++i)
                    aw[s % WD][kk][i] = __builtin_bit_cast(bf16x8, __builtin_amdgcn_raw_buffer_load_b128(rw, wvo, ((s * 2 + kk) * WM + i) * 1024, 0));
        };
#pragma unroll
        for (int s = 0; s < WD; ++s) load_w(s);
        f32x4 sva[3], svb[3];
        int soffa, soffb;
        item_issue(cur, tid_l, 1, 2, 4 * IPP, sva, soffa);
        item_issue(cur, tid_l + NT, 1, 2, 4 * IPP, svb, soffb);
        __syncthreads();

        f32x16 acc[WM][WN];
#pragma unroll
        for (int i = 0; i < WM; ++i)
#pragma unroll
            for (int j = 0; j < WN; ++j)
#pragma unroll
                for (int r = 0; r < 16; ++r) acc[i][j][r] = 0.f;
        bf16x8 bv[2][2][WN];
        auto read_ops = [&](int set, int s) {
            const int dt = s / 7, dh = s - dt * 7;
#pragma unroll
            for (int kk = 0; kk < 2; ++kk)
#pragma unroll
                for (int j = 0; j < WN; ++j)
                    bv[set][kk][j] = *reinterpret_cast<const bf16x8*>(patch + xbase[j] + (dt * NR + dh) * PITCH + kk * 32);
        };
        read_ops(0, 0);
        static_for<0, STEPS>([&](auto step) {
            constexpr int s = decltype(step)::value;
            constexpr int set = s & 1;
            if (s + 1 < STEPS) read_ops(set ^ 1, s + 1);
            __builtin_amdgcn_sched_barrier(0);
#pragma unroll
            for (int kk = 0; kk < 2; ++kk)
#pragma unroll
                for (int i = 0; i < WM; ++i)
#pragma unroll
                    for (int j = 0; j < WN; ++j)
                        acc[i][j] = __builtin_amdgcn_mfma_f32_32x32x16_bf16(aw[s % WD][kk][i], bv[set][kk][j], acc[i][j], 0, 0, 0);
            if (s + WD < STEPS) load_w(s + WD);
            __builtin_amdgcn_sched_barrier(0);
            if (s == 1) { item_commit(sva, soffa); item_issue(cur, tid_l + 2 * NT, 1, 2, 4 * IPP, sva, soffa); }
            if (s == 3) { item_commit(svb, soffb); item_issue(cur, tid_l, 8, 1, 5 * IPP, svb, soffb); }
            if (s == 5) { item_commit(sva, soffa); item_issue(cur, tid_l + NT, 8, 1, 5 * IPP, sva, soffa); }
            if (s == 7) { item_commit(svb, soffb); item_issue(cur, tid_l + 2 * NT, 8, 1, 5 * IPP, svb, soffb); }
            if (s == 9) { item_commit(sva, soffa); item_issue(cur, tid_l + 3 * NT, 8, 1, 5 * IPP, sva, soffa); }
            if (s == 11) item_commit(svb, soffb);
            if (s == 13) item_commit(sva, soffa);
            if (s == 5 || s == 9 || s == 13) __syncthreads();
        });
        const TileAt done = cur;
        auto prefetch_next = [&]() {
            cur = tile_at(min(work + 1, w_end - 1));
#pragma unroll
            for (int u = 0; u < 3; ++u) item_issue(cur, tid_l + NT * u, 0, 2, 4 * IPP, pv[u], poff[u]);
        };
        __syncthreads();
        const int64_t pbase = (int64_t)done.b * a.y_bs + ((int64_t)(done.to0 + lt) * a.Ho + done.ho0) * WO + (wave & 1) * WPOS;
        const bool relu = a.relu != 0;
        if (a.half) {
            unsigned short* yh = reinterpret_cast<unsigned short*>(a.out) + pbase;
            unsigned char* tile = patch + wave * (BM * EPI_PITCH);
            f32x4 ss[WM][4][2];
#pragma unroll
            for (int i = 0; i < WM; ++i)
#pragma unroll
                for (int q = 0; q < 4; ++q)
#pragma unroll
                    for (int u = 0; u < 2; ++u)
                        ss[i][q][u] = *reinterpret_cast<const f32x4*>(rows + 2 * (i * 32 + 8 * q + 4 * (lane_l >> 5)) + 4 * u);
#pragma unroll
            for (int i = 0; i < WM; ++i)
#pragma unroll
                for (int q = 0; q < 4; ++q)
#pragma unroll
                    for (int rr = 0; rr < 4; ++rr) {
                        const float sc = ss[i][q][rr >> 1][2 * (rr & 1)], sh = ss[i][q][rr >> 1][2 * (rr & 1) + 1];
#pragma unroll
                        for (int j = 0; j < WN; ++j) {
                            float v = acc[i][j][4 * q + rr] * sc + sh;
                            if (relu) v = fmaxf(v, 0.f);
                            *reinterpret_cast<unsigned short*>(tile + (i * 32 + 8 * q + 4 * (lane_l >> 5) + rr) * EPI_PITCH + (j * 32 + (lane_l & 31)) * 2) =
                                (unsigned short)(cvt_pk_bf16(v, 0.f) & 0xffffu);
                        }
                    }
            __builtin_amdgcn_sched_barrier(0);
            prefetch_next();
            __builtin_amdgcn_sched_barrier(0);
#pragma unroll
            for (int u = 0; u < BM * 12 / 64; ++u) {
                const int p = lane_l + 64 * u;
                const int row = p / 12, c = p - row * 12;
                if (m0 + row < a.M) {
                    const Words4 v = *reinterpret_cast<const Words4*>(tile + row * EPI_PITCH + c * 16);
                    *reinterpret_cast<Words4*>(yh + (int64_t)(m0 + row) * a.y_cs + c * 8) = v;
                }
            }
        } else {
            float* yf = reinterpret_cast<float*>(a.out) + pbase;
#pragma unroll
            for (int i = 0; i < WM; ++i)
#pragma unroll
                for (int r = 0; r < 16; ++r) {
                    const int lr = i * 32 + (r & 3) + 8 * (r >> 2) + 4 * (lane_l >> 5);
                    const float sc = rows[2 * lr], sh = rows[2 * lr + 1];
                    if (m0 + lr >= a.M) continue;
#pragma unroll
                    for (int j = 0; j < WN; ++j) {
                        float v = acc[i][j][r] * sc + sh;
                        if (relu) v = fmaxf(v, 0.f);
                        yf[(int64_t)(m0 + lr) * a.y_cs + j * 32 + (lane_l & 31)] = v;
                    }
                }
            prefetch_next();
        }
        __syncthreads();
        if (work + 1 < w_end) begin_tile(cur, tid_l);
    }
}

__global__ __launch_bounds__(256) void pack_conv1a_operand_order_kernel(unsigned* __restrict__ wp, const float* __restrict__ w, int M, int pairs) {
    for (int p = blockIdx.x * 256 + threadIdx.x; p < pairs; p += gridDim.x * 256) {
        const int e2 = p & 3, ln = (p >> 2) & 63, i = (p >> 8) & 1, kk = (p >> 9) & 1, rest = p >> 10;
        const int s = rest % STEPS, blk = rest / STEPS;
        const int m = blk * BM + i * 32 + (ln & 31);
        float v[2];
#pragma unroll
        for (int u = 0; u < 2; ++u) {
            const int k = kk * 16 + (ln >> 5) * 8 + e2 * 2 + u, dw = k >> 2, ci = k & 3;
            v[u] = (m < M && dw < 7 && ci < 3) ? w[((int64_t)m * 3 + ci) * 343 + s * 7 + dw] : 0.f;
        }
        wp[p] = cvt_pk_bf16(v[0], v[1]);
    }
}

}

int otal_conv::launch_conv1a_tile(const Conv1aTileArgs& a, void* ws, size_t ws_bytes, hipStream_t st) {
    if ((2 * a.x_cs + (int64_t)a.Ti * a.Hi * 96) * 4 >= (1LL << 31)) return OTAL_E_UNSUPPORTED;
    const int tm = (a.M + BM - 1) / BM;
    const size_t wb = (size_t)tm * BM * STEPS * 64;
    if (!ws || ws_bytes < wb) return OTAL_E_UNSUPPORTED;
    const int pairs = tm * BM * STEPS * 16;
    hipLaunchKernelGGL(pack_conv1a_operand_order_kernel, dim3((pairs + 255) / 256), dim3(256), 0, st, reinterpret_cast<unsigned*>(ws), a.w, a.M, pairs);
    if (int e = otal_launch_status()) return e;
    Conv1aTileArgs t = a;
    t.wp = reinterpret_cast<const unsigned short*>(ws);
    const int nwork = a.B * (a.To / TT) * (a.Ho / TR) * tm;
    int ncu = OTAL_OPT("OTAL_CONV_1A_WGS");
    if (ncu <= 0) {
        static int cus = 0;
        if (!cus) {
            int dev = 0, n = 0;
            if (hipGetDevice(&dev) != hipSuccess || hipDeviceGetAttribute(&n, hipDeviceAttributeMultiprocessorCount, dev) != hipSuccess || n <= 0) n = 256;
            cus = n;
        }
        ncu = cus;
    }
    const int per_wg = (nwork + ncu - 1) / ncu;
    const int nwg = (nwork + per_wg - 1) / per_wg;
    hipLaunchKernelGGL(conv1a_tile_fwd_kernel, dim3(nwg), dim3(NT), 0, st, t, nwork, per_wg, tm);
    return otal_launch_status();
}
```

opental_amd/csrc/conv_select.h:

```cpp
#pragma once
#include <initializer_list>
#include <stddef.h>
#include <stdint.h>
#include "conv_index.h"
#include "options.h"

namespace {

enum { MODE_FWD = 0, MODE_DGRAD = 1, MODE_WGRAD = 2 };

constexpr int C1_TT = 2, C1_TR = 2, C1_WO = 48;
constexpr int C1T_TT = 4, C1T_TR = 4;
constexpr int C1_STEPS = 49;
constexpr int W1_TC = 128;
constexpr int PJ_HW = 36;
constexpr int PW_KS = 32;
constexpr size_t TAB_PAD = 64;
constexpr int CHUNK_PAD = 16;
constexpr int PTAB_PAD = 64;

static inline size_t align256(size_t v) { return (v + 255) & ~(size_t)255; }
static inline size_t tab_bytes(int K) { return (((size_t)K + TAB_PAD) * (2 * sizeof(int)) + 255) & ~(size_t)255; }
static inline int chunk_kp(int K) { return (K + 31) / 32 * 32; }
static inline size_t chunk_tab_bytes(int K) { return align256(((size_t)chunk_kp(K) / 8 + CHUNK_PAD) * (2 * sizeof(int))); }
static inline size_t chunk_wp_bytes(int M, int BM, int K) {
    return align256(((size_t)((M + BM - 1) / BM * BM) * chunk_kp(K) + 64) * sizeof(unsigned short));
}
static inline size_t ptab_bytes(const ConvGeom& g, int cw) {
    return align256(((size_t)g.B * conv_out_positions(g) / cw + PTAB_PAD) * (2 * sizeof(int)));
}
static inline size_t conv1a_wp_bytes(int M) { return align256((size_t)((M + 63) / 64 * 64) * C1_STEPS * 64); }
static inline int64_t gather_extent_bytes(const ConvGeom& g, int mode, int esz = 4) {
    if (mode == MODE_FWD) return esz * ((int64_t)(g.B - 1) * g.x_bs + (int64_t)(g.Cin - 1) * g.x_cs + conv_in_positions(g));
    return esz * ((int64_t)(g.B - 1) * g.y_bs + (int64_t)(g.Cout - 1) * g.y_cs + conv_out_positions(g));
}

static inline int choose_bm(int M, bool tall = false) {
    if (tall && M % 192 == 0) return 192;
    const int cand[4] = {128, 96, 64, 32};
    const double pen[4] = {1.00, 1.03, 1.10, 1.30};
    int best = 128;
    double bc = 1e30;
    for (int i = 0; i < 4; ++i) {
        const double c = (double)((M + cand[i] - 1) / cand[i] * cand[i]) * pen[i];
        if (c < bc) { bc = c; best = cand[i]; }
    }
    return best;
}

static inline int choose_splits(int tiles, int K, int prec = 1, bool wgrad = false) {
    const bool wv = wgrad && prec;
    const int target = wv ? 2048 : 512;
    const int minsteps = wv ? 16 : (prec ? 8 : 4);
    const int cap = wv ? 1024 : 384;
    if (tiles >= target * 3 / 4) return 1;
    int want = (target + tiles - 1) / tiles;
    int maxs = K / (minsteps * 32);
    if (maxs < 1) maxs = 1;
    int s = want < maxs ? want : maxs;
    return s < 1 ? 1 : (s > cap ? cap : s);
}

static inline int generic_wgrad_splits(int tiles, int K) {
    const int ms = 4;
    const int tg = 512;
    int want = (tg + tiles - 1) / tiles, maxs = K / (ms * 32);
    if (maxs < 1) maxs = 1;
    const int s = tiles >= tg * 3 / 4 ? 1 : (want < maxs ? want : maxs);
    return s > 384 ? 384 : s;
}
static inline int wgrad1x1_mt(int M) {
    const int cand[3] = {4, 3, 2};
    int mt = 2, best = 1 << 30;
    for (int i = 0; i < 3; ++i) {
        const int rb = cand[i] * 32, blocks = (M + rb - 1) / rb;
        const int cost = blocks * 256 + blocks * rb;
        if (cost < best) { best = cost; mt = cand[i]; }
    }
    return mt;
}
static inline int wgrad1x1_splits(int mt, int tiles, int K) {
    const int wgs = (mt <= 2 ? 2 : 1) * 256;
    int splits = tiles >= wgs ? 1 : wgs / tiles;
    if (splits > K / (8 * 32)) splits = K / (8 * 32) > 0 ? K / (8 * 32) : 1;
    return splits;
}
static inline int wgrad_direct_rows(const ConvGeom& g) { return g.Wi == 24 ? (g.Hi % 8 == 0 ? 8 : 4) : g.Wi; }
struct WgradDirectShape { int BM, steps, want; };
static inline WgradDirectShape wgrad_direct_shape(const ConvGeom& g, int M) {
    WgradDirectShape d;
    const bool planes6 = g.Wi == 6, planes3 = g.Wi == 3;
    d.BM = planes6 || planes3 ? 32 : 64;
    d.steps = planes3 ? g.B * (g.Ti / 16) : planes6 ? g.B * (g.Ti / 4) : g.B * g.Ti * (g.Hi / wgrad_direct_rows(g));
    const int tiles = (M + d.BM - 1) / d.BM * ((g.Cin + 31) / 32);
    int splits = tiles >= 256 ? 1 : 256 / tiles;
    const int target = OTAL_OPT("OTAL_WDIRECT_BLOCKS");
    if (target > 0) splits = target / tiles > 0 ? target / tiles : 1;
    const int min_steps = planes3 || planes6 ? 4 : 8;
    if (splits > d.steps / min_steps) splits = d.steps / min_steps > 0 ? d.steps / min_steps : 1;
    d.want = splits;
    return d;
}
static inline int conv1a_wgrad_blocks(const ConvGeom& g) { return g.B * (g.To / 2) * (g.Ho / 2); }
static inline int conv1a_wgrad_splits(int nblocks) {
    const int splits = OTAL_OPT("OTAL_W1A_SPLITS") > 0 ? OTAL_OPT("OTAL_W1A_SPLITS") : 73;
    return splits > nblocks ? nblocks : splits;
}
static inline int proj_fwd_splits(int Cin, int tiles) {
    int splits = (512 + tiles - 1) / tiles;
    while (splits > 1 && (Cin % (4 * splits) != 0)) --splits;
    return splits;
}
static inline int wgrad1d_upw(int units) { return units >= 8 ? 4 : units >= 4 ? 2 : 1; }

static inline bool conv1a_half_out_ok(const ConvGeom& g, const void* y) {
    return g.y_bs % 8 == 0 && g.y_cs % 8 == 0 && (reinterpret_cast<uintptr_t>(y) & 15) == 0;
}
static inline bool conv1a_direct_eligible(const ConvGeom& g, int mode, int prec, const void* x) {
    if (!prec || mode != MODE_FWD || g.nlev > 1 || OTAL_OPT("OTAL_CONV_NO1A")) return false;
    if (g.Cin != 3 || g.kt != 7 || g.kh != 7 || g.kw != 7 || g.st != 2 || g.sh != 2 || g.sw != 2) return false;
    if (g.pt != 2 || g.ph != 2 || g.pw != 2 || g.Wi != 96 || g.Wo != C1_WO || g.Hi != 2 * g.Ho || g.Ti != 2 * g.To) return false;
    if (g.To % C1_TT || g.Ho % C1_TR || g.x_bs % 4 || g.x_cs % 4 || (reinterpret_cast<uintptr_t>(x) & 15)) return false;
    return (int64_t)g.B * g.To * g.Ho * g.Wo < (1LL << 31);
}
static inline int conv1a_tile_eligible(int To, int Ho) {
    return To % C1T_TT == 0 && Ho % C1T_TR == 0 && !OTAL_OPT("OTAL_CONV_1A_NOTILE");
}
static inline bool conv1a_wgrad_eligible(const ConvGeom& g, int prec, const void* x, const void* dy) {
    if (!prec || g.nlev > 1 || OTAL_OPT("OTAL_CONV_NO1AW")) return false;
    if (g.Cin != 3 || g.Cout > 64 || g.kt != 7 || g.kh != 7 || g.kw != 7 || g.st != 2 || g.sh != 2 || g.sw != 2) return false;
    if (g.pt != 2 || g.ph != 2 || g.pw != 2 || g.Wi != 96 || g.Wo != C1_WO || g.Hi != 2 * g.Ho || g.Ti != 2 * g.To) return false;
    if (g.To % 2 || g.Ho % 2 || g.x_bs % 4 || g.x_cs % 4 || g.y_bs % 4 || g.y_cs % 4) return false;
    if ((reinterpret_cast<uintptr_t>(x) & 15) || (reinterpret_cast<uintptr_t>(dy) & 15)) return false;
    const int64_t ex = gather_extent_bytes(g, MODE_FWD), ey = gather_extent_bytes(g, MODE_DGRAD);
    return ex > 0 && ey > 0 && ex < (1LL << 31) && ey < (1LL << 31);
}

static inline bool proj_fwd_eligible(const ConvGeom& g, int mode, int prec, const void* x, const void* w) {
    if (!prec || mode != MODE_FWD || g.nlev > 1 || OTAL_OPT("OTAL_CONV_NOPROJ")) return false;
    if (g.kt != 1 || g.st != 1 || g.kh != g.Hi || g.kw != g.Wi || g.Ho != 1 || g.Wo != 1 || g.To != g.Ti) return false;
    if (g.Hi * g.Wi != PJ_HW || g.ph != 0 || g.pw != 0 || g.pt != 0 || g.Cin % 4) return false;
    if (((uintptr_t)x & 3) || ((uintptr_t)w & 3)) return false;
    const int64_t ex = gather_extent_bytes(g, MODE_FWD), ew = 4 * (int64_t)g.Cout * g.Cin * PJ_HW;
    return ex > 0 && ex < (1LL << 31) && ew < (1LL << 31);
}
static inline bool proj_wgrad_eligible(const ConvGeom& g, int prec, const void* x, const void* dy) {
    if (!prec || g.nlev > 1 || OTAL_OPT("OTAL_CONV_NOPROJW")) return false;
    if (g.kt != 1 || g.st != 1 || g.kh != g.Hi || g.kw != g.Wi || g.Ho != 1 || g.Wo != 1 || g.To != g.Ti) return false;
    if (g.ph != 0 || g.pw != 0 || g.pt != 0 || g.Hi * g.Wi < 2) return false;
    if (g.To % PW_KS || g.y_cs < g.To || (g.y_cs & 3) || (g.y_bs & 3)) return false;
    if (((uintptr_t)x & 15) || ((uintptr_t)dy & 15) || (g.x_bs & 3) || (g.x_cs & 3)) return false;
    const int64_t ex = gather_extent_bytes(g, MODE_FWD), ey = gather_extent_bytes(g, MODE_DGRAD);
    const int64_t eo = 4 * (int64_t)g.Cout * g.Cin * g.Hi * g.Wi;
    return ex > 0 && ey > 0 && ex < (1LL << 31) && ey < (1LL << 31) && eo < (1LL << 31);
}

static inline bool conv1d_tile_eligible(const ConvGeom& g, int mode, int prec, const void* src, bool emask) {
    if (!prec || mode == MODE_WGRAD || OTAL_OPT("OTAL_CONV_NO1DTILE")) return false;
    if (g.Hi != 1 || g.Wi != 1 || g.Ho != 1 || g.Wo != 1 || g.kh != 1 || g.kw != 1 || g.st != 1 || g.To != g.Ti) return false;
    if (!((g.kt == 1 && g.pt == 0) || (g.kt == 3 && g.pt == 1))) return false;
    if (g.Ti > 4096) return false;
    if ((mode == MODE_FWD ? g.Cout : g.Cin) > 2048) return false;
    const int C = mode == MODE_FWD ? g.Cin : g.Cout;
    if (C % 128) return false;
    if (mode == MODE_DGRAD && emask) return false;
    if (((uintptr_t)src & 3)) return false;
    const int64_t ext = gather_extent_bytes(g, mode);
    return ext > 0 && ext < (1LL << 31);
}
static inline int wgrad1d_chunks(const ConvGeom& g) { return (g.Ti + W1_TC - 1) / W1_TC; }
static inline bool wgrad1d_eligible(const ConvGeom& g, int prec, const void* x, const void* dy) {
    if (!prec || OTAL_OPT("OTAL_CONV_NOW1D")) return false;
    if (g.Hi != 1 || g.Wi != 1 || g.Ho != 1 || g.Wo != 1 || g.kh != 1 || g.kw != 1 || g.st != 1 || g.To != g.Ti) return false;
    if (!((g.kt == 1 && g.pt == 0) || (g.kt == 3 && g.pt == 1))) return false;
    if (g.Cin % 64 || (g.x_bs | g.x_cs | g.y_bs | g.y_cs) & 1) return false;
    if ((reinterpret_cast<uintptr_t>(x) | reinterpret_cast<uintptr_t>(dy)) & 7) return false;
    return (int64_t)g.B * wgrad1d_chunks(g) <= 1024;
}

static inline bool chunk_eligible(const ConvGeom& g, int mode, int prec) {
    if (!prec || mode == MODE_WGRAD) return false;
    const int C = mode == MODE_FWD ? g.Cin : g.Cout;
    if (C % 8 && !(mode == MODE_FWD && g.kw >= 3)) return false;
    const int64_t ext = gather_extent_bytes(g, mode);
    return ext > 0 && ext < (int64_t)0xfffffff0u;
}
static inline bool conv1x1_stream_eligible(const ConvGeom& g, int mode) {
    if (OTAL_OPT("OTAL_CONV_NO1X1STREAM")) return false;
    if (g.kt != 1 || g.kh != 1 || g.kw != 1 || g.st != 1 || g.sh != 1 || g.sw != 1 || g.nlev > 1) return false;
    const int64_t P = conv_out_positions(g);
    if (P != conv_in_positions(g) || P % 128) return false;
    const int C = mode == MODE_FWD ? g.Cin : g.Cout;
    return C % 8 == 0;
}

static inline int direct_bm(const ConvGeom& g, int M) {
    if (M % 96 == 0) return 96;
    if (M > 96) {
        const int64_t nt = (int64_t)g.B * conv_out_positions(g) / 256;
        const int64_t w64 = (M + 63) / 64 * nt, w96 = (M + 95) / 96 * nt;
        if (w64 <= 512 && (w96 + 255) / 256 * 96 < (w64 + 255) / 256 * 64) return 96;
    }
    if (M % 64 == 0) return 64;
    if (M <= 32) return 32;
    const int pad64 = (M + 63) / 64 * 64;
    return (pad64 - M) * 100 <= M * 34 ? 64 : 0;
}
static inline int direct_bnp(const ConvGeom& g, int M) {
    const int BM = direct_bm(g, M);
    if (!BM) return 0;
    const int64_t tm = (M + BM - 1) / BM, NP = (int64_t)g.B * conv_out_positions(g);
    const int min_tiles = OTAL_OPT("OTAL_CONV_DIRECT_MINTILES");
    if (BM == 96 && conv_out_positions(g) % 512 == 0 && tm * (NP / 512) >= OTAL_OPT("OTAL_CONV_DIRECT_MINTILES512")) return 512;
    if (tm * (NP / 256) >= min_tiles) return 256;
    if (tm * (NP / 128) >= min_tiles) return 128;
    return 0;
}
static inline bool direct_eligible(const ConvGeom& g, int mode, int prec, int M) {
    if (OTAL_OPT("OTAL_CONV_NODIRECT") || !prec || mode == MODE_WGRAD || g.nlev > 1) return false;
    if (g.kt != 3 || g.kh != 3 || g.kw != 3 || g.st != 1 || g.sh != 1 || g.sw != 1 || g.pt != 1 || g.ph != 1 || g.pw != 1) return false;
    if (g.To != g.Ti || g.Ho != g.Hi || g.Wo != g.Wi || g.Wi > 24) return false;
    const int P = conv_out_positions(g);
    const int C = mode == MODE_FWD ? g.Cin : g.Cout;
    if (P % 256 || C % 16 || !direct_bnp(g, M)) return false;
    const int64_t ext = gather_extent_bytes(g, mode);
    return ext > 0 && ext < (1LL << 31);
}
static inline size_t direct_wp_bytes(const ConvGeom& g, int M, int C) {
    const int BM = direct_bm(g, M);
    return align256((size_t)((M + BM - 1) / BM * BM) * C * 27 * 2 + 1024);
}

static inline bool wgrad_direct_eligible(const ConvGeom& g, int prec, const void* x, const void* dy) {
    if (!prec || OTAL_OPT("OTAL_CONV_NOWDIRECT") || g.nlev > 1) return false;
    if (g.kt != 3 || g.kh != 3 || g.kw != 3 || g.st != 1 || g.sh != 1 || g.sw != 1 || g.pt != 1 || g.ph != 1 || g.pw != 1) return false;
    if (g.To != g.Ti || g.Ho != g.Hi || g.Wo != g.Wi) return false;
    const bool planes6 = g.Wi == 6 && g.Hi == 6 && g.Ti % 4 == 0;
    const bool planes3 = g.Wi == 3 && g.Hi == 3 && g.Ti % 16 == 0;
    if (!((g.Wi == 24 && g.Hi % 4 == 0) || (g.Wi == 12 && g.Hi == 12) || planes6 || planes3) || g.Cin % 2) return false;
    if (g.Cin < (planes3 ? 32 : 64) || g.Cout < 64) return false;
    if (((uintptr_t)x & 15) || ((uintptr_t)dy & 15) || g.x_cs % 4 || g.x_bs % 4 || g.y_cs % 4 || g.y_bs % 4) return false;
    const int64_t ex = gather_extent_bytes(g, MODE_FWD), ey = gather_extent_bytes(g, MODE_DGRAD);
    return ex > 0 && ey > 0 && ex < (1LL << 31) && ey < (1LL << 31);
}
static inline bool wgrad1x1_wide_eligible(const ConvGeom& g, int prec, const void* x, const void* dy) {
    if (!prec || g.nlev > 1 || OTAL_OPT("OTAL_CONV_NOW1X1")) return false;
    if (g.kt != 1 || g.kh != 1 || g.kw != 1 || g.st != 1 || g.sh != 1 || g.sw != 1) return false;
    if (g.To != g.Ti || g.Ho != g.Hi || g.Wo != g.Wi) return false;
    if (g.Hi == 1 && g.Wi == 1) return false;
    if (conv_out_positions(g) % 32 || (int64_t)g.Cout * g.Cin > (1 << 20)) return false;
    if (((uintptr_t)x & 3) || ((uintptr_t)dy & 3)) return false;
    const int64_t ex = gather_extent_bytes(g, MODE_FWD), ey = gather_extent_bytes(g, MODE_DGRAD);
    return ex > 0 && ey > 0 && ex < (1LL << 31) && ey < (1LL << 31);
}
static inline bool wgrad_pair_mode(const ConvGeom& g, int prec) {
    if (!prec || g.nlev > 1) return false;
    if (g.sw != 2 || g.st > 2 || g.sh > 2 || g.kw > 7 || g.pw > 3 || g.Wo % 8 || conv_out_positions(g) % 32) return false;
    if (g.Wi - (2 * (g.Wo - 8) - g.pw + 6) < 12) return false;
    const int64_t ex = 4 * ((int64_t)(g.B - 1) * g.x_bs + (int64_t)(g.Cin - 1) * g.x_cs + conv_in_positions(g));
    const int64_t ey = 4 * ((int64_t)(g.B - 1) * g.y_bs + (int64_t)(g.Cout - 1) * g.y_cs + conv_out_positions(g));
    return ex > 0 && ey > 0 && ex < (int64_t)0xffffff00u && ey < (int64_t)0xfffffff0u;
}
static inline int wgrad_vector_width(const ConvGeom& g, int prec) {
    if (!prec) return 0;
    if (g.st != 1 || g.sh != 1 || g.sw != 1 || g.nlev > 1) return 0;
    if (g.To != g.Ti || g.Ho != g.Hi || g.Wo != g.Wi) return 0;
    if ((g.kw != 1 && g.kw != 3) || g.pw != (g.kw - 1) / 2) return 0;
    if (conv_out_positions(g) % 32) return 0;
    const int64_t ex = 4 * ((int64_t)(g.B - 1) * g.x_bs + (int64_t)(g.Cin - 1) * g.x_cs + conv_in_positions(g));
    const int64_t ey = 4 * ((int64_t)(g.B - 1) * g.y_bs + (int64_t)(g.Cout - 1) * g.y_cs + conv_out_positions(g));
    if (ex <= 0 || ey <= 0 || ex >= (int64_t)0xfffffff0u || ey >= (int64_t)0xfffffff0u) return 0;
    if (g.kt == 1 && g.kh == 1 && g.kw == 1) return 8;
    if (g.Wi % 8 == 0) return 8;
    if (g.Wi % 4 == 0) return 4;
    if (g.Wi % 2 == 0) return 2;
    return 0;
}

enum ConvKernel {
    CK_GENERIC,
    CK_PROJ, CK_CONV1A, CK_CONV1D_TILE, CK_DIRECT, CK_CHUNKED,
    CK_CONV1A_WGRAD, CK_PROJ_WGRAD, CK_WGRAD_DIRECT, CK_WGRAD1X1, CK_WGRAD_VECTOR, CK_WGRAD1D,
};
static inline const char* conv_kernel_name(int kernel) {
    switch (kernel) {
        case CK_GENERIC: return "generic";
        case CK_PROJ: return "proj";
        case CK_CONV1A: return "conv1a";
        case CK_CONV1D_TILE: return "conv1d_tile";
        case CK_DIRECT: return "direct";
        case CK_CHUNKED: return "chunked";
        case CK_CONV1A_WGRAD: return "conv1a_wgrad";
        case CK_PROJ_WGRAD: return "proj_wgrad";
        case CK_WGRAD_DIRECT: return "wgrad_direct";
        case CK_WGRAD1X1: return "wgrad1x1_wide";
        case CK_WGRAD_VECTOR: return "vector";
        case CK_WGRAD1D: return "wgrad1d";
    }
    return "?";
}
enum ConvPrologue { PRO_NONE = 0, PRO_CHUNK = 1, PRO_PTAB = 2, PRO_DIRECT = 3 };

struct ConvQuery {
    ConvGeom g;
    int mode;
    int precision;
    int accumulate;
    int has_mask;
    uintptr_t x, w, dy, out, mask;
    uintptr_t prologue, prologue2;
    int pair;
};
struct ConvStep {
    int kernel;
    int cw;
    bool next;
};
struct ConvPlan {
    int n;
    ConvStep step[8];
    int prologue;
};

static inline int conv_step_prologue(int kernel) {
    switch (kernel) {
        case CK_CONV1D_TILE: case CK_CHUNKED: return PRO_CHUNK;
        case CK_DIRECT: return PRO_DIRECT;
        case CK_WGRAD_VECTOR: return PRO_PTAB;
        default: return PRO_NONE;
    }
}

static inline int conv_prologue_layout(const ConvGeom& g, int mode, int prec) {
    if (mode == MODE_WGRAD) return wgrad_pair_mode(g, prec) || wgrad_vector_width(g, prec) ? PRO_PTAB : PRO_NONE;
    if (proj_fwd_eligible(g, mode, prec, nullptr, nullptr)) return PRO_NONE;
    if (conv1a_direct_eligible(g, mode, prec, nullptr)) return PRO_NONE;
    if (direct_eligible(g, mode, prec, mode == MODE_FWD ? g.Cout : g.Cin)) return PRO_DIRECT;
    return chunk_eligible(g, mode, prec) ? PRO_CHUNK : PRO_NONE;
}
static inline void conv_plan_half(const ConvQuery& q, ConvPlan& p) {
    const ConvGeom& g = q.g;
    const void* px = (const void*)(q.mode == MODE_DGRAD ? q.out : q.x);
    const void* py = (const void*)(q.mode == MODE_FWD ? q.out : q.dy);
    auto add = [&p](int kernel, bool next, int cw = 0) { p.step[p.n++] = ConvStep{kernel, cw, next}; };
    if (!(q.precision & 1) || !(q.precision & 4) || q.accumulate) return;
    if (((uintptr_t)px | (uintptr_t)py) & 15) return;
    if (q.mode == MODE_DGRAD && q.has_mask && (!(q.precision & 16) || (q.mask & 15))) return;
    if (g.nlev > 1) return;
    if (conv_out_positions(g) % 8 || conv_in_positions(g) % 8 || g.x_bs % 8 || g.x_cs % 8 || g.y_bs % 8 || g.y_cs % 8) return;
    if (q.mode == MODE_FWD || q.mode == MODE_DGRAD) {
        const int M = q.mode == MODE_FWD ? g.Cout : g.Cin, C = q.mode == MODE_FWD ? g.Cin : g.Cout;
        if (direct_eligible(g, q.mode, 1, M) && !(g.Wi & 1)) add(CK_DIRECT, false);
        else if (chunk_eligible(g, q.mode, 1) && C % 8 == 0 && conv_in_positions(g) == conv_out_positions(g)) add(CK_CHUNKED, false);
        return;
    }
    const int cw = wgrad_vector_width(g, 1);
    if (wgrad_direct_eligible(g, 1, px, py)) add(CK_WGRAD_DIRECT, true);
    else if (wgrad1x1_wide_eligible(g, 1, px, py)) add(CK_WGRAD1X1, true);
    if (cw) add(CK_WGRAD_VECTOR, false, cw);
}

static inline ConvPlan conv_plan(const ConvQuery& q) {
    ConvPlan p = {};
    const ConvGeom& g = q.g;
    const int prec = q.precision & 1, half = (q.precision >> 2) & 1;
    p.prologue = conv_prologue_layout(g, q.mode, prec);
    if (q.precision & 8) { conv_plan_half(q, p); return p; }
    const void *x = (const void*)q.x, *w = (const void*)q.w, *dy = (const void*)q.dy, *out = (const void*)q.out;
    auto add = [&p](int kernel, bool next, int cw = 0) { p.step[p.n++] = ConvStep{kernel, cw, next}; };
    if (q.mode == MODE_WGRAD) {
        if (conv1a_wgrad_eligible(g, prec, x, dy) && (!half || g.y_bs % 8 + g.y_cs % 8 == 0)) add(CK_CONV1A_WGRAD, !half);
        if (half) return p;
        if (proj_wgrad_eligible(g, prec, x, dy)) add(CK_PROJ_WGRAD, true);
        if (wgrad_direct_eligible(g, prec, x, dy)) add(CK_WGRAD_DIRECT, true);
        if (wgrad1x1_wide_eligible(g, prec, x, dy)) add(CK_WGRAD1X1, true);
        if (wgrad_pair_mode(g, prec)) { add(CK_WGRAD_VECTOR, false, 8); return p; }
        if (const int cw = wgrad_vector_width(g, prec)) { add(CK_WGRAD_VECTOR, false, cw); return p; }
        if (wgrad1d_eligible(g, prec, x, dy)) add(CK_WGRAD1D, true);
        add(CK_GENERIC, false);
        return p;
    }
    const int M = q.mode == MODE_FWD ? g.Cout : g.Cin;
    if (q.mode == MODE_FWD) {
        if (proj_fwd_eligible(g, q.mode, prec, x, w)) add(CK_PROJ, true);
        if (half) {
            if (conv1a_direct_eligible(g, q.mode, prec, x) && conv1a_half_out_ok(g, out)) add(CK_CONV1A, false);
            else if (direct_eligible(g, q.mode, prec, M) && conv1a_half_out_ok(g, out)) add(CK_DIRECT, false);
            return p;
        }
        if (conv1a_direct_eligible(g, q.mode, prec, x)) { add(CK_CONV1A, false); return p; }
    }
    if (half) return p;
    if (conv1d_tile_eligible(g, q.mode, prec, q.mode == MODE_FWD ? x : dy, q.has_mask)) add(CK_CONV1D_TILE, true);
    if (direct_eligible(g, q.mode, prec, M)) add(CK_DIRECT, false);
    else if (chunk_eligible(g, q.mode, prec)) add(CK_CHUNKED, false);
    else add(CK_GENERIC, false);
    return p;
}

static inline int conv_half_storage(const ConvGeom& g, int mode, int precision) {
    if (!(precision & 1) || g.y_bs % 8 || g.y_cs % 8) return 0;
    ConvQuery q = {};
    q.g = g;
    q.mode = mode;
    q.precision = precision | 4;
    const ConvPlan p = conv_plan(q);
    for (int i = 0; i < p.n; ++i)
        if (p.step[i].kernel != CK_PROJ) return 1;
    return 0;
}

}
struct ConvLaunchShape {
    size_t front_bytes;
    size_t second_at;
    int N, K;
    int bm, tm, tn, grid[3];
    int units, splits, per_split;
    size_t slab_bytes;
    bool refuse;
};
namespace {

static inline size_t shape_take(ConvLaunchShape& s, size_t& left, size_t n) {
    if (left < n) s.refuse = true; else left -= n;
    return n;
}
static inline void fit_splits(ConvLaunchShape& s, int M, int want, int units, int round, const void* ws, size_t ws_bytes, bool all_or_none = false) {
    const size_t slab1 = (size_t)M * s.N * sizeof(float);
    if (!ws) ws_bytes = 0;
// ... 128 lines not shown
```

opental_amd/csrc/options.h:

```cpp
#pragma once

struct OtalOption { const char* name; int dflt; };
constexpr OtalOption OTAL_OPTIONS[] = {
    {"OTAL_CONV_1A_NOTILE", 0},           {"OTAL_CONV_1A_WGS", 0},
    {"OTAL_CONV_DIRECT_MINTILES", 140},   {"OTAL_CONV_DIRECT_MINTILES512", 512},
    {"OTAL_CONV_DIRECT_XPF2", 3},         {"OTAL_CONV_NO1A", 0},
    {"OTAL_CONV_NO1AW", 0},               {"OTAL_CONV_NO1DTILE", 0},
    {"OTAL_CONV_NO1X1STREAM", 0},         {"OTAL_CONV_NODIRECT", 0},
    {"OTAL_CONV_NOPROJ", 0},              {"OTAL_CONV_NOPROJW", 0},
    {"OTAL_CONV_NOW1D", 0},               {"OTAL_CONV_NOW1X1", 0},
    {"OTAL_CONV_NOWDIRECT", 0},           {"OTAL_LOSS_NOSTAGE", 0},
    {"OTAL_POOL_NO133", 0},               {"OTAL_POOL_NOROWS", 0},
    {"OTAL_W1A_SPLITS", 0},               {"OTAL_WDIRECT_BLOCKS", 0},
};
constexpr int OTAL_NUM_OPTIONS = sizeof(OTAL_OPTIONS) / sizeof(OTAL_OPTIONS[0]);
constexpr bool otal_streq(const char* a, const char* b) { return *a == *b && (*a == 0 || otal_streq(a + 1, b + 1)); }
constexpr int otal_option_index(const char* name, int i = 0) {
    return i == OTAL_NUM_OPTIONS ? -1 : otal_streq(OTAL_OPTIONS[i].name, name) ? i : otal_option_index(name, i + 1);
}
int* otal_option_slot(int index);
#define OTAL_OPT(name) ([]() -> int {                                                                              \
    constexpr int index_ = otal_option_index(name);                                                              \
    static_assert(index_ >= 0, "unknown option " name " (options.h: OTAL_OPTIONS)");                               \
    static int* const slot_ = otal_option_slot(index_);                                                          \
    return *slot_;                                                                                               \
}())
```

Baseline: 1007.

## Fuse conv1a with the following 1x3x3 maxpool in the tile kernel epilogue

Adds a fused conv1a+maxpool(1,3,3)/(1,2,2) path. The MFMA tile kernel, compiled a second time with a pool epilogue, writes pooled outputs, argmax taps and sign bits directly, so the full-resolution conv1a activation is never written to or read back from memory. The Python backbone uses it when conv1a is half-output and followed by the pool, and passes a stand-in tensor in place of the unpooled activation. The work split is regrouped into column-per-workgroup order so row-tile carries across the pooling window can be kept, which may reduce load balance and adds epilogue complexity.

```diff
diff --git a/include/opental_hip.h b/include/opental_hip.h
--- a/include/opental_hip.h
+++ b/include/opental_hip.h
@@ -80,6 +80,11 @@
 int otal_conv_flush_reduces(void* stream);
 
 const char* otal_conv_last_kernel(void);
+
+int otal_conv1a_pool_taken(const int* geom);
+int otal_conv1a_pool_fwd(const int* geom, const int64_t* strides, const float* x, const float* w, const float* scale,
+                         const float* shift, void* y, int y_f32, unsigned char* argtap, unsigned char* signbits, int relu,
+                         int precision, void* ws, size_t ws_bytes, void* stream);
 
 int otal_conv_pack_wt(const float* w, float* wt, int Cout, int Cin, int kvol, void* stream);
 
diff --git a/opental_amd/common/i3d_backbone.py b/opental_amd/common/i3d_backbone.py
--- a/opental_amd/common/i3d_backbone.py
+++ b/opental_amd/common/i3d_backbone.py
@@ -332,6 +332,7 @@
         cur_scale = None
         BF = torch.bfloat16
         need_grad = any(ctx.needs_input_grad)
+        fused_pool = None
         raw_out = {e[1:] for e in endpoints if e.startswith("=")}
         endpoints = tuple(e.lstrip("=") for e in endpoints)
 
@@ -367,12 +368,23 @@
                         and ops.half_storage_ok(2, tuple(cur.shape), weights[wi].shape[0], k, s)):
                     half = True
                 half_grads[si + 1] = grad_half
-                y = ops.conv_forward(cur, weights[wi], k, s, scale=sc(wi), shift=sh(wi), relu=True, half_out=half)
+                y = None
+                if half and si == 0 and pooled_next:
+                    yshape = (cur.shape[0], weights[wi].shape[0]) + tuple(ops._out_positions(cur, weights[wi].shape[0], k, s, None, False))
+                    chain1 = _step_half_ok(plan[1], yshape, weights)
+                    if chain1 or (yshape[3] % 2 == 0 and yshape[4] % 4 == 0):
+                        fused_pool = ops.conv1a_pool_forward(cur, weights[wi], k, s, scale=sc(wi), shift=sh(wi), half_out=chain1)
+                        if fused_pool is not None:
+                            y = fused_pool[3]
+                if y is None:
+                    y = ops.conv_forward(cur, weights[wi], k, s, scale=sc(wi), shift=sh(wi), relu=True, half_out=half)
                 tape.append(("conv", wi, k, s, cur, y, cur_scale, sc(wi)))
                 cur, cur_scale = y, sc(wi)
             elif kind == "pool":
                 _, k, s, _ = step
-                if chain:
+                if si == 1 and fused_pool is not None:
+                    y, arg, bits = fused_pool[:3]
+                elif chain:
                     y, arg, bits = ops.maxpool3d_forward(cur, k, s, signbits=True, half_out=True)
                 elif cur_scale is not None:
                     y, arg, bits = ops.maxpool3d_forward(cur, k, s, signbits=True)
diff --git a/opental_amd/common/ops.py b/opental_amd/common/ops.py
--- a/opental_amd/common/ops.py
+++ b/opental_amd/common/ops.py
@@ -648,6 +648,37 @@
                                   prec | 12, pre, wsp, wsn, L.stream()), "otal_conv_fwd (bf16 tensors)")
     _prof_end(ev, "fwd", g)
     return out
+
+
+def conv1a_pool_forward(x, w, k, s, scale=None, shift=None, half_out=True, signbits=True, force=False):
+    k, s = _k3(k), _k3(s)
+    if x.dtype != torch.float32 or x.dim() != 5 or int(CONV_PRECISION) != 1 or not w.is_contiguous():
+        return None
+    Cout = w.shape[0]
+    B, Cin, Ti, Hi, Wi = x.shape
+    g, outn = _make_geom(B, Cin, Cout, (Ti, Hi, Wi), k, s, None, False)
+    lib = L.lib()
+    ga = (ctypes.c_int * len(g))(*g)
+    if not force and not lib.otal_conv1a_pool_taken(ga):
+        return None
+    pooln = (outn[0], -(-outn[1] // 2), -(-outn[2] // 2))
+    _check(x, "x")
+    y = torch.empty((B, Cout) + pooln, dtype=torch.bfloat16 if half_out else torch.float32, device=x.device)
+    arg = torch.empty((B, Cout) + pooln, dtype=torch.uint8, device=x.device) if signbits else None
+    bits = torch.empty(B * Cout * pooln[0] * pooln[1] * (outn[2] // 4), dtype=torch.uint8, device=x.device) if signbits else None
+    xb, xc = _bs(x)
+    yb, yc = _bs(y)
+    sa = (ctypes.c_int64 * 4)(xb, xc, yb, yc)
+    wsp, wsn = _ws_args(x.device)
+    ev = _prof_begin()
+    rc = lib.otal_conv1a_pool_fwd(ga, sa, L.ptr(x), L.ptr(w), _opt(scale), _opt(shift), L.ptr(y), int(not half_out), _opt(arg),
+                                  _opt(bits), 1, int(CONV_PRECISION) | 4, wsp, wsn, L.stream())
+    if rc == L.E_UNSUPPORTED:
+        return None
+    L.check(rc, "otal_conv1a_pool_fwd")
+    _prof_end(ev, "fwd", g)
+    standin = torch.empty(1, dtype=torch.bfloat16, device=x.device).expand((B, Cout) + outn)
+    return y, arg, bits, standin
 
 
 def pack_wt(w):
diff --git a/opental_amd/csrc/conv1a_tile.h b/opental_amd/csrc/conv1a_tile.h
--- a/opental_amd/csrc/conv1a_tile.h
+++ b/opental_amd/csrc/conv1a_tile.h
@@ -19,4 +19,14 @@
 
 __attribute__((visibility("hidden"))) int launch_conv1a_tile(const Conv1aTileArgs& a, void* ws, size_t ws_bytes, hipStream_t st);
 
+struct Conv1aPoolArgs {
+    void* y;
+    unsigned char* arg;
+    unsigned char* signbits;
+    int64_t y_bs, y_cs;
+    int y_f32;
+};
+__attribute__((visibility("hidden"))) int launch_conv1a_tile_pool(const Conv1aTileArgs& a, const Conv1aPoolArgs& p, void* ws, size_t ws_bytes,
+                                                                  hipStream_t st);
+
 }
diff --git a/opental_amd/csrc/conv1a_tile.hip b/opental_amd/csrc/conv1a_tile.hip
--- a/opental_amd/csrc/conv1a_tile.hip
+++ b/opental_amd/csrc/conv1a_tile.hip
@@ -41,217 +41,105 @@
     int b, to0, ho0, mblk;
 };
 
-__global__ __launch_bounds__(NT) void conv1a_tile_fwd_kernel(const otal_conv::Conv1aTileArgs a, int nwork, int per_wg, int tm) {
-    __shared__ __attribute__((aligned(16))) unsigned char patch[NPL * PLANE];
-    __shared__ __attribute__((aligned(16))) float rows[2 * BM];
-    const int tid = threadIdx.x, lane = tid & 63;
-    const int wave = __builtin_amdgcn_readfirstlane(tid >> 6);
-    const int tiles_h = a.Ho / TR, tiles_t = a.To / TT;
-    int wg = blockIdx.x;
-    if ((gridDim.x & 7) == 0) wg = (wg & 7) * (gridDim.x >> 3) + (wg >> 3);
-    const int w_begin = wg * per_wg, w_end = min(nwork, w_begin + per_wg);
-    if (w_begin >= w_end) return;
-    auto tile_at = [&](int w) {
-        TileAt t;
-        t.mblk = w % tm; w /= tm;
-        const int th = w % tiles_h; w /= tiles_h;
-        t.to0 = (w % tiles_t) * TT;
-        t.b = w / tiles_t;
-        t.ho0 = th * TR;
-        return t;
-    };
-    const unsigned cs_bytes = (unsigned)(a.x_cs * 4);
-    const int x_extent = (int)((2 * a.x_cs + (int64_t)a.Ti * a.Hi * 96) * 4);
-
-    auto item_issue = [&](const TileAt& t, int e, int pl0, int plstep, int nitems, f32x4 (&v)[3], int& off) {
-        const auto rx = __builtin_amdgcn_make_buffer_rsrc(const_cast<float*>(a.x + (int64_t)t.b * a.x_bs), 0, x_extent, 0x00020000);
-        const bool live = e < nitems;
-        const int gi = e / IPP, rem = e - gi * IPP, rr = rem / QPR, q = rem - rr * QPR;
-        const int pl = pl0 + plstep * gi;
-        const int ti = 2 * t.to0 - 2 + pl, hi = 2 * t.ho0 - 2 + rr;
-        const bool ok = live && (unsigned)ti < (unsigned)a.Ti && (unsigned)hi < (unsigned)a.Hi;
-        const bool ld = ok;
-        off = live ? pl * PLANE + rr * PITCH + (4 * q + 2) * 8 : -1;
-        const unsigned vo = ld ? (unsigned)((((int64_t)ti * a.Hi + hi) * 96 + 4 * q) * 4) : 0xffffffffu;
-#pragma unroll
-        for (int ci = 0; ci < 3; ++ci)
-            v[ci] = __builtin_bit_cast(f32x4, __builtin_amdgcn_raw_buffer_load_b128(rx, vo, ci * cs_bytes, 0));
-    };
-    auto item_commit = [&](const f32x4 (&v)[3], int off) {
-        if (off < 0) return;
-        u32x4 lo, hi;
-        lo[0] = cvt_pk_bf16(v[0][0], v[1][0]); lo[1] = cvt_pk_bf16(v[2][0], 0.f);
-        lo[2] = cvt_pk_bf16(v[0][1], v[1][1]); lo[3] = cvt_pk_bf16(v[2][1], 0.f);
-        hi[0] = cvt_pk_bf16(v[0][2], v[1][2]); hi[1] = cvt_pk_bf16(v[2][2], 0.f);
-        hi[2] = cvt_pk_bf16(v[0][3], v[1][3]); hi[3] = cvt_pk_bf16(v[2][3], 0.f);
-        *reinterpret_cast<u32x4*>(patch + off) = lo;
-        *reinterpret_cast<u32x4*>(patch + off + 16) = hi;
-    };
-
-    const auto rw = __builtin_amdgcn_make_buffer_rsrc(const_cast<unsigned short*>(a.wp), 0, (int)((int64_t)tm * BM * STEPS * 64), 0x00020000);
-    constexpr int WD = 2;
-
-    const int lt = wave >> 1;
-    int xbase[WN];
-#pragma unroll
-    for (int j = 0; j < WN; ++j) {
-        const int o = (wave & 1) * WPOS + j * 32 + (lane & 31);
-        const int lr = o / WO, wo = o - lr * WO;
-        xbase[j] = ((2 * lt) * NR + 2 * lr) * PITCH + (2 * wo) * 8 + (lane >> 5) * 16;
-    }
-
-    f32x4 pv[3][3];
-    int poff[3];
-    TileAt cur = tile_at(w_begin);
-#pragma unroll
-    for (int u = 0; u < 3; ++u) item_issue(cur, tid + NT * u, 0, 2, 4 * IPP, pv[u], poff[u]);
-
-    auto begin_tile = [&](const TileAt& t, int tid_l) {
-        if (tid_l < BM) {
-            const int m = t.mblk * BM + tid_l;
-            rows[2 * tid_l] = (m < a.M && a.scale) ? a.scale[m] : 1.f;
-            rows[2 * tid_l + 1] = (m < a.M && a.shift) ? a.shift[m] : 0.f;
-        }
-        for (int i = tid_l; i < NPL * NR * 6; i += NT) {
-            const int row = i / 6, e = i - row * 6;
-            *reinterpret_cast<Words2*>(patch + row * PITCH + (e < 2 ? e : 96 + e) * 8) = Words2{0u, 0u};
-        }
-#pragma unroll
-        for (int u = 0; u < 3; ++u) item_commit(pv[u], poff[u]);
-    };
-    begin_tile(cur, tid);
-
-    for (int work = w_begin; work < w_end; ++work) {
-        const int m0 = cur.mblk * BM;
-        int tid_l = tid;
-        asm volatile("" : "+v"(tid_l));
-        const int lane_l = tid_l & 63;
-        const unsigned wvo = (unsigned)(cur.mblk * (BM * STEPS * 64) + lane * 16);
-        bf16x8 aw[WD][2][WM];
-        auto load_w = [&](int s) {
-#pragma unroll
-            for (int kk = 0; kk < 2; ++kk)
-#pragma unroll
-                for (int i = 0; i < WM; ++i)
-                    aw[s % WD][kk][i] = __builtin_bit_cast(bf16x8, __builtin_amdgcn_raw_buffer_load_b128(rw, wvo, ((s * 2 + kk) * WM + i) * 1024, 0));
-        };
-#pragma unroll
-        for (int s = 0; s < WD; ++s) load_w(s);
-        f32x4 sva[3], svb[3];
-        int soffa, soffb;
-        item_issue(cur, tid_l, 1, 2, 4 * IPP, sva, soffa);
-        item_issue(cur, tid_l + NT, 1, 2, 4 * IPP, svb, soffb);
-        __syncthreads();
-
-        f32x16 acc[WM][WN];
-#pragma unroll
-        for (int i = 0; i < WM; ++i)
-#pragma unroll
-            for (int j = 0; j < WN; ++j)
-#pragma unroll
-                for (int r = 0; r < 16; ++r) acc[i][j][r] = 0.f;
-        bf16x8 bv[2][2][WN];
-        auto read_ops = [&](int set, int s) {
-            const int dt = s / 7, dh = s - dt * 7;
-#pragma unroll
-            for (int kk = 0; kk < 2; ++kk)
-#pragma unroll
-                for (int j = 0; j < WN; ++j)
-                    bv[set][kk][j] = *reinterpret_cast<const bf16x8*>(patch + xbase[j] + (dt * NR + dh) * PITCH + kk * 32);
-        };
-        read_ops(0, 0);
-        static_for<0, STEPS>([&](auto step) {
-            constexpr int s = decltype(step)::value;
-            constexpr int set = s & 1;
-            if (s + 1 < STEPS) read_ops(set ^ 1, s + 1);
-            __builtin_amdgcn_sched_barrier(0);
-#pragma unroll
-            for (int kk = 0; kk < 2; ++kk)
-#pragma unroll
-                for (int i = 0; i < WM; ++i)
-#pragma unroll
-                    for (int j = 0; j < WN; ++j)
-                        acc[i][j] = __builtin_amdgcn_mfma_f32_32x32x16_bf16(aw[s % WD][kk][i], bv[set][kk][j], acc[i][j], 0, 0, 0);
-            if (s + WD < STEPS) load_w(s + WD);
-            __builtin_amdgcn_sched_barrier(0);
-            if (s == 1) { item_commit(sva, soffa); item_issue(cur, tid_l + 2 * NT, 1, 2, 4 * IPP, sva, soffa); }
-            if (s == 3) { item_commit(svb, soffb); item_issue(cur, tid_l, 8, 1, 5 * IPP, svb, soffb); }
-            if (s == 5) { item_commit(sva, soffa); item_issue(cur, tid_l + NT, 8, 1, 5 * IPP, sva, soffa); }
-            if (s == 7) { item_commit(svb, soffb); item_issue(cur, tid_l + 2 * NT, 8, 1, 5 * IPP, svb, soffb); }
-            if (s == 9) { item_commit(sva, soffa); item_issue(cur, tid_l + 3 * NT, 8, 1, 5 * IPP, sva, soffa); }
-            if (s == 11) item_commit(svb, soffb);
-            if (s == 13) item_commit(sva, soffa);
-            if (s == 5 || s == 9 || s == 13) __syncthreads();
-        });
-        const TileAt done = cur;
-        auto prefetch_next = [&]() {
-            cur = tile_at(min(work + 1, w_end - 1));
-#pragma unroll
-            for (int u = 0; u < 3; ++u) item_issue(cur, tid_l + NT * u, 0, 2, 4 * IPP, pv[u], poff[u]);
-        };
-        __syncthreads();
-        const int64_t pbase = (int64_t)done.b * a.y_bs + ((int64_t)(done.to0 + lt) * a.Ho + done.ho0) * WO + (wave & 1) * WPOS;
-        const bool relu = a.relu != 0;
-        if (a.half) {
-            unsigned short* yh = reinterpret_cast<unsigned short*>(a.out) + pbase;
-            unsigned char* tile = patch + wave * (BM * EPI_PITCH);
-            f32x4 ss[WM][4][2];
-#pragma unroll
-            for (int i = 0; i < WM; ++i)
-#pragma unroll
-                for (int q = 0; q < 4; ++q)
-#pragma unroll
-                    for (int u = 0; u < 2; ++u)
-                        ss[i][q][u] = *reinterpret_cast<const f32x4*>(rows + 2 * (i * 32 + 8 * q + 4 * (lane_l >> 5)) + 4 * u);
-#pragma unroll
-            for (int i = 0; i < WM; ++i)
-#pragma unroll
-                for (int q = 0; q < 4; ++q)
-#pragma unroll
-                    for (int rr = 0; rr < 4; ++rr) {
-                        const float sc = ss[i][q][rr >> 1][2 * (rr & 1)], sh = ss[i][q][rr >> 1][2 * (rr & 1) + 1];
-#pragma unroll
-                        for (int j = 0; j < WN; ++j) {
-                            float v = acc[i][j][4 * q + rr] * sc + sh;
-                            if (relu) v = fmaxf(v, 0.f);
-                            *reinterpret_cast<unsigned short*>(tile + (i * 32 + 8 * q + 4 * (lane_l >> 5) + rr) * EPI_PITCH + (j * 32 + (lane_l & 31)) * 2) =
-                                (unsigned short)(cvt_pk_bf16(v, 0.f) & 0xffffu);
-                        }
-                    }
-            __builtin_amdgcn_sched_barrier(0);
-            prefetch_next();
-            __builtin_amdgcn_sched_barrier(0);
-#pragma unroll
-            for (int u = 0; u < BM * 12 / 64; ++u) {
-                const int p = lane_l + 64 * u;
-                const int row = p / 12, c = p - row * 12;
-                if (m0 + row < a.M) {
-                    const Words4 v = *reinterpret_cast<const Words4*>(tile + row * EPI_PITCH + c * 16);
-                    *reinterpret_cast<Words4*>(yh + (int64_t)(m0 + row) * a.y_cs + c * 8) = v;
-                }
+using PoolOut = otal_conv::Conv1aPoolArgs;
+
+__device__ __forceinline__ void pool_row_words(const unsigned char* p, bool ninth, unsigned (&W)[5]) {
+    const Words4 v = *reinterpret_cast<const Words4*>(p);
+    W[0] = v.a & 0x7fff7fffu; W[1] = v.b & 0x7fff7fffu; W[2] = v.c & 0x7fff7fffu; W[3] = v.d & 0x7fff7fffu;
+    W[4] = ninth ? ((unsigned)*reinterpret_cast<const unsigned short*>(p + 16) & 0x7fffu) : 0u;
+}
+template <int DH>
+__device__ __forceinline__ void pool_row_keys(const unsigned (&W)[5], unsigned (&best)[4], bool first) {
+#pragma unroll
+    for (int o = 0; o < 4; ++o) {
+        const unsigned c0 = (W[o] << 16) | (unsigned)(15 - (DH * 3 + 0));
+        const unsigned c1 = (W[o] & 0xffff0000u) | (unsigned)(15 - (DH * 3 + 1));
+        const unsigned c2 = (W[o + 1] << 16) | (unsigned)(15 - (DH * 3 + 2));
+        const unsigned m = max(max(c0, c1), c2);
+        best[o] = first ? m : max(best[o], m);
+    }
+}
+__device__ __forceinline__ unsigned pool_sign_nibbles(const unsigned (&W)[5]) {
+    unsigned acc = 0u;
+#pragma unroll
+    for (int k = 0; k < 4; ++k) acc |= ((W[k] & 0xffffu) ? 1u : 0u) << (2 * k) | ((W[k] >> 16) ? 2u : 0u) << (2 * k);
+    return acc;
+}
+__device__ __forceinline__ void pool_store(const PoolOut& po, const unsigned (&best)[4], int64_t bm, int64_t yoff, int64_t plane_rows,
+                                           int hp, int c) {
+    const int64_t p = (plane_rows + hp) * 24 + 4 * c;
+    if (po.y_f32) {
+        *reinterpret_cast<u32x4*>(reinterpret_cast<float*>(po.y) + yoff + p) =
+            u32x4{best[0] & 0xffff0000u, best[1] & 0xffff0000u, best[2] & 0xffff0000u, best[3] & 0xffff0000u};
+    } else {
+        *reinterpret_cast<Words2*>(reinterpret_cast<unsigned short*>(po.y) + yoff + p) =
+            Words2{__builtin_amdgcn_perm(best[1], best[0], 0x07060302u), __builtin_amdgcn_perm(best[3], best[2], 0x07060302u)};
+    }
+    if (po.arg) {
+        const unsigned lows = __builtin_amdgcn_perm(best[1], best[0], 0x0c0c0400u) | __builtin_amdgcn_perm(best[3], best[2], 0x04000c0cu);
+        *reinterpret_cast<unsigned*>(po.arg + bm + p) = 0x0f0f0f0fu - lows;
+    }
+}
+
+__device__ __forceinline__ void pool_epilogue(const otal_conv::Conv1aTileArgs& a, const PoolOut& po, const unsigned char* patch,
+                                              unsigned* carry, const TileAt& done, int m0, int wave, int lane_l) {
+    const int lt = wave >> 1, odd = wave & 1;
+    const int Hp = a.Ho >> 1, hp = (done.ho0 >> 1) + odd;
+    const bool col_first = done.ho0 == 0, col_last = done.ho0 + TR == a.Ho;
+    const unsigned char* own = patch + wave * (BM * EPI_PITCH);
+    const unsigned char* other = patch + (wave ^ 1) * (BM * EPI_PITCH);
+    const int64_t plane_rows = (int64_t)(done.to0 + lt) * Hp;
+#pragma unroll
+    for (int u = 0; u < BM * 6 / 64; ++u) {
+        const int p = lane_l + 64 * u;
+        const int row = p / 6, c = p - row * 6;
+        const int m = m0 + row;
+        if (m >= a.M) continue;
+        const bool ninth = c < 5;
+        unsigned W0[5], W1[5], W2[5];
+        pool_row_words(own + row * EPI_PITCH + c * 16, ninth, W0);
+        pool_row_words(own + row * EPI_PITCH + WO * 2 + c * 16, ninth, W1);
+        pool_row_words(other + row * EPI_PITCH + c * 16, ninth, W2);
+        const int64_t bm = ((int64_t)done.b * a.M + m) * a.To * Hp * 24;
+        const int64_t yoff = (int64_t)done.b * po.y_bs + (int64_t)m * po.y_cs;
+        unsigned best[4], third[4];
+        pool_row_keys<0>(W0, best, true);
+        pool_row_keys<1>(W1, best, false);
+        pool_row_keys<2>(W2, third, true);
+        unsigned* cw = carry + (lt * BM + row) * 24 + 4 * c;
+        if (!odd) {
+#pragma unroll
+            for (int o = 0; o < 4; ++o) best[o] = max(best[o], third[o]);
+            pool_store(po, best, bm, yoff, plane_rows, hp, c);
+        } else {
+            if (!col_first) {
+                const u32x4 k = *reinterpret_cast<const u32x4*>(cw);
+#pragma unroll
+                for (int o = 0; o < 4; ++o) third[o] = max(third[o], k[o]);
+                pool_store(po, third, bm, yoff, plane_rows, hp - 2, c);
             }
-        } else {
-            float* yf = reinterpret_cast<float*>(a.out) + pbase;
-#pragma unroll
-            for (int i = 0; i < WM; ++i)
-#pragma unroll
-                for (int r = 0; r < 16; ++r) {
-                    const int lr = i * 32 + (r & 3) + 8 * (r >> 2) + 4 * (lane_l >> 5);
-                    const float sc = rows[2 * lr], sh = rows[2 * lr + 1];
-                    if (m0 + lr >= a.M) continue;
-#pragma unroll
-                    for (int j = 0; j < WN; ++j) {
-                        float v = acc[i][j][r] * sc + sh;
-                        if (relu) v = fmaxf(v, 0.f);
-                        yf[(int64_t)(m0 + lr) * a.y_cs + j * 32 + (lane_l & 31)] = v;
-                    }
-                }
-            prefetch_next();
-        }
-        __syncthreads();
-        if (work + 1 < w_end) begin_tile(cur, tid_l);
-    }
-}
+            if (col_last) pool_store(po, best, bm, yoff, plane_rows, hp, c);
+            else *reinterpret_cast<u32x4*>(cw) = u32x4{best[0], best[1], best[2], best[3]};
+        }
+        if (po.signbits) {
+            const unsigned r0 = pool_sign_nibbles(W0), r1 = pool_sign_nibbles(W1);
+            const unsigned b0 = (r0 & 15u) | ((r1 & 15u) << 4), b1 = (r0 >> 4) | (r1 & 0xf0u);
+            *reinterpret_cast<unsigned short*>(po.signbits + ((((int64_t)done.b * a.M + m) * a.To + done.to0 + lt) * Hp + hp) * 12 + 2 * c) =
+                (unsigned short)(b0 | (b1 << 8));
+        }
+    }
+}
+
+#define C1T_KERNEL conv1a_tile_fwd_kernel
+#define C1T_POOL 0
+#include "conv1a_tile_kernel.inc"
+#undef C1T_KERNEL
+#undef C1T_POOL
+#define C1T_KERNEL conv1a_tile_pool_fwd_kernel
+#define C1T_POOL 1
+#include "conv1a_tile_kernel.inc"
+#undef C1T_KERNEL
+#undef C1T_POOL
 
 __global__ __launch_bounds__(256) void pack_conv1a_operand_order_kernel(unsigned* __restrict__ wp, const float* __restrict__ w, int M, int pairs) {
     for (int p = blockIdx.x * 256 + threadIdx.x; p < pairs; p += gridDim.x * 256) {
@@ -268,19 +156,7 @@
     }
 }
 
-}
-
-int otal_conv::launch_conv1a_tile(const Conv1aTileArgs& a, void* ws, size_t ws_bytes, hipStream_t st) {
-    if ((2 * a.x_cs + (int64_t)a.Ti * a.Hi * 96) * 4 >= (1LL << 31)) return OTAL_E_UNSUPPORTED;
-    const int tm = (a.M + BM - 1) / BM;
-    const size_t wb = (size_t)tm * BM * STEPS * 64;
-    if (!ws || ws_bytes < wb) return OTAL_E_UNSUPPORTED;
-    const int pairs = tm * BM * STEPS * 16;
-    hipLaunchKernelGGL(pack_conv1a_operand_order_kernel, dim3((pairs + 255) / 256), dim3(256), 0, st, reinterpret_cast<unsigned*>(ws), a.w, a.M, pairs);
-    if (int e = otal_launch_status()) return e;
-    Conv1aTileArgs t = a;
-    t.wp = reinterpret_cast<const unsigned short*>(ws);
-    const int nwork = a.B * (a.To / TT) * (a.Ho / TR) * tm;
+int persistent_wgs() {
     int ncu = OTAL_OPT("OTAL_CONV_1A_WGS");
     if (ncu <= 0) {
         static int cus = 0;
@@ -291,8 +167,81 @@
         }
         ncu = cus;
     }
+    return ncu;
+}
+
+int pack_weights(const otal_conv::Conv1aTileArgs& a, int tm, void* ws, size_t ws_bytes, hipStream_t st) {
+    if ((2 * a.x_cs + (int64_t)a.Ti * a.Hi * 96) * 4 >= (1LL << 31)) return OTAL_E_UNSUPPORTED;
+    const size_t wb = (size_t)tm * BM * STEPS * 64;
+    if (!ws || ws_bytes < wb) return OTAL_E_UNSUPPORTED;
+    const int pairs = tm * BM * STEPS * 16;
+    hipLaunchKernelGGL(pack_conv1a_operand_order_kernel, dim3((pairs + 255) / 256), dim3(256), 0, st, reinterpret_cast<unsigned*>(ws), a.w, a.M, pairs);
+    return otal_launch_status();
+}
+
+}
+
+int otal_conv::launch_conv1a_tile(const Conv1aTileArgs& a, void* ws, size_t ws_bytes, hipStream_t st) {
+    const int tm = (a.M + BM - 1) / BM;
+    if (int e = pack_weights(a, tm, ws, ws_bytes, st)) return e;
+    Conv1aTileArgs t = a;
+    t.wp = reinterpret_cast<const unsigned short*>(ws);
+    const int nwork = a.B * (a.To / TT) * (a.Ho / TR) * tm;
+    const int ncu = persistent_wgs();
     const int per_wg = (nwork + ncu - 1) / ncu;
     const int nwg = (nwork + per_wg - 1) / per_wg;
     hipLaunchKernelGGL(conv1a_tile_fwd_kernel, dim3(nwg), dim3(NT), 0, st, t, nwork, per_wg, tm);
     return otal_launch_status();
 }
+
+int otal_conv::launch_conv1a_tile_pool(const Conv1aTileArgs& a, const Conv1aPoolArgs& p, void* ws, size_t ws_bytes, hipStream_t st) {
+    if (!a.relu || !a.half || a.To % TT || a.Ho % TR) return OTAL_E_UNSUPPORTED;
+    const int tm = (a.M + BM - 1) / BM;
+    if (int e = pack_weights(a, tm, ws, ws_bytes, st)) return e;
+    Conv1aTileArgs t = a;
+    t.wp = reinterpret_cast<const unsigned short*>(ws);
+    t.out = nullptr;
+    const Conv1aPoolLaunch l = conv1a_pool_launch(a.B, a.To, a.Ho, a.M, persistent_wgs());
+    hipLaunchKernelGGL(conv1a_tile_pool_fwd_kernel, dim3(l.nwg), dim3(NT), 0, st, t, p, l.columns * l.tiles_h, l.per_wg, tm);
+    return otal_launch_status();
+}
+
+namespace {
+int conv1a_pool_geometry(const int* d) {
+    for (int i = 0; i < 15; ++i) if (d[i] <= 0) return OTAL_E_SHAPE;
+    if (d[1] != 3 || d[9] != 7 || d[10] != 7 || d[11] != 7 || d[12] != 2 || d[13] != 2 || d[14] != 2) return OTAL_E_UNSUPPORTED;
+    if (d[15] != 2 || d[16] != 2 || d[17] != 2 || d[18] > 1 || d[5] != 96 || d[8] != WO) return OTAL_E_UNSUPPORTED;
+    if (d[3] != 2 * d[6] || d[4] != 2 * d[7] || d[6] % TT || d[7] % TR) return OTAL_E_UNSUPPORTED;
+    if ((int64_t)d[0] * d[6] * d[7] * WO >= (1LL << 31) || (int64_t)d[2] * d[6] * d[7] * WO >= (1LL << 31)) return OTAL_E_UNSUPPORTED;
+    return 0;
+}
+}
+
+extern "C" int otal_conv1a_pool_taken(const int* geom) {
+    if (!geom) return 0;
+    const int mode = OTAL_OPT("OTAL_CONV_1A_POOL");
+    if (mode <= 0 || OTAL_OPT("OTAL_CONV_NO1A") || OTAL_OPT("OTAL_CONV_1A_NOTILE") || conv1a_pool_geometry(geom)) return 0;
+    return mode >= 2 || conv1a_pool_taken(geom[0], geom[6], geom[7], geom[2], persistent_wgs());
+}
+
+extern "C" int otal_conv1a_pool_fwd(const int* geom, const int64_t* strides, const float* x, const float* w, const float* scale,
+                                    const float* shift, void* y, int y_f32, unsigned char* argtap, unsigned char* signbits, int relu,
+                                    int precision, void* ws, size_t ws_bytes, void* stream) {
+    g_layer_kernel = "";
+    if (!geom || !strides || !x || !w || !y) return OTAL_E_NULL;
+    if (int e = conv1a_pool_geometry(geom)) return e;
+    if (!relu || precision != 5) return OTAL_E_UNSUPPORTED;
+    otal_conv::Conv1aTileArgs t = {};
+    t.x = x; t.w = w; t.scale = scale; t.shift = shift;
+    t.x_bs = strides[0]; t.x_cs = strides[1];
+    t.B = geom[0]; t.Ti = geom[3]; t.Hi = geom[4]; t.To = geom[6]; t.Ho = geom[7]; t.M = geom[2];
+    t.relu = 1; t.half = 1;
+    otal_conv::Conv1aPoolArgs p = {};
+    p.y = y; p.arg = argtap; p.signbits = signbits; p.y_bs = strides[2]; p.y_cs = strides[3]; p.y_f32 = y_f32 ? 1 : 0;
+    if (t.x_bs % 4 || t.x_cs % 4 || (reinterpret_cast<uintptr_t>(x) & 15) || p.y_bs % 4 || p.y_cs % 4 ||
+        (reinterpret_cast<uintptr_t>(y) & 15) || (reinterpret_cast<uintptr_t>(argtap) & 3) || (reinterpret_cast<uintptr_t>(signbits) & 1))
+        return OTAL_E_UNSUPPORTED;
+    const int e = otal_conv::launch_conv1a_tile_pool(t, p, ws, ws_bytes, (hipStream_t)stream);
+    if (e) return e;
+    return otal_layer_launched("conv1a_tile_pool_fwd");
+}
diff --git a/opental_amd/csrc/conv1a_tile_kernel.inc b/opental_amd/csrc/conv1a_tile_kernel.inc
--- /dev/null
+++ b/opental_amd/csrc/conv1a_tile_kernel.inc
@@ -0,0 +1,237 @@
+#if C1T_POOL
+__global__ __launch_bounds__(NT) void C1T_KERNEL(const otal_conv::Conv1aTileArgs a, const PoolOut po, int nwork, int per_wg, int tm) {
+#else
+__global__ __launch_bounds__(NT) void C1T_KERNEL(const otal_conv::Conv1aTileArgs a, int nwork, int per_wg, int tm) {
+#endif
+    __shared__ __attribute__((aligned(16))) unsigned char patch[NPL * PLANE];
+    __shared__ __attribute__((aligned(16))) float rows[2 * BM];
+#if C1T_POOL
+    __shared__ __attribute__((aligned(16))) unsigned carry[TT * BM * 24];
+#endif
+    const int tid = threadIdx.x, lane = tid & 63;
+    const int wave = __builtin_amdgcn_readfirstlane(tid >> 6);
+    const int tiles_h = a.Ho / TR, tiles_t = a.To / TT;
+    int wg = blockIdx.x;
+    if ((gridDim.x & 7) == 0) wg = (wg & 7) * (gridDim.x >> 3) + (wg >> 3);
+    const int w_begin = wg * per_wg, w_end = min(nwork, w_begin + per_wg);
+    if (w_begin >= w_end) return;
+    auto tile_at = [&](int w) {
+        TileAt t;
+#if C1T_POOL
+        const int th = w % tiles_h; w /= tiles_h;
+        t.mblk = w % tm; w /= tm;
+#else
+        t.mblk = w % tm; w /= tm;
+        const int th = w % tiles_h; w /= tiles_h;
+#endif
+        t.to0 = (w % tiles_t) * TT;
+        t.b = w / tiles_t;
+        t.ho0 = th * TR;
+        return t;
+    };
+    const unsigned cs_bytes = (unsigned)(a.x_cs * 4);
+    const int x_extent = (int)((2 * a.x_cs + (int64_t)a.Ti * a.Hi * 96) * 4);
+
+    auto item_issue = [&](const TileAt& t, int e, int pl0, int plstep, int nitems, f32x4 (&v)[3], int& off) {
+        const auto rx = __builtin_amdgcn_make_buffer_rsrc(const_cast<float*>(a.x + (int64_t)t.b * a.x_bs), 0, x_extent, 0x00020000);
+        const bool live = e < nitems;
+        const int gi = e / IPP, rem = e - gi * IPP, rr = rem / QPR, q = rem - rr * QPR;
+        const int pl = pl0 + plstep * gi;
+        const int ti = 2 * t.to0 - 2 + pl, hi = 2 * t.ho0 - 2 + rr;
+        const bool ok = live && (unsigned)ti < (unsigned)a.Ti && (unsigned)hi < (unsigned)a.Hi;
+        const bool ld = ok;
+        off = live ? pl * PLANE + rr * PITCH + (4 * q + 2) * 8 : -1;
+        const unsigned vo = ld ? (unsigned)((((int64_t)ti * a.Hi + hi) * 96 + 4 * q) * 4) : 0xffffffffu;
+#pragma unroll
+        for (int ci = 0; ci < 3; ++ci)
+            v[ci] = __builtin_bit_cast(f32x4, __builtin_amdgcn_raw_buffer_load_b128(rx, vo, ci * cs_bytes, 0));
+    };
+    auto item_commit = [&](const f32x4 (&v)[3], int off) {
+        if (off < 0) return;
+        u32x4 lo, hi;
+        lo[0] = cvt_pk_bf16(v[0][0], v[1][0]); lo[1] = cvt_pk_bf16(v[2][0], 0.f);
+        lo[2] = cvt_pk_bf16(v[0][1], v[1][1]); lo[3] = cvt_pk_bf16(v[2][1], 0.f);
+        hi[0] = cvt_pk_bf16(v[0][2], v[1][2]); hi[1] = cvt_pk_bf16(v[2][2], 0.f);
+        hi[2] = cvt_pk_bf16(v[0][3], v[1][3]); hi[3] = cvt_pk_bf16(v[2][3], 0.f);
+        *reinterpret_cast<u32x4*>(patch + off) = lo;
+        *reinterpret_cast<u32x4*>(patch + off + 16) = hi;
+    };
+
+    const auto rw = __builtin_amdgcn_make_buffer_rsrc(const_cast<unsigned short*>(a.wp), 0, (int)((int64_t)tm * BM * STEPS * 64), 0x00020000);
+    constexpr int WD = 2;
+
+    const int lt = wave >> 1;
+    int xbase[WN];
+#pragma unroll
+    for (int j = 0; j < WN; ++j) {
+        const int o = (wave & 1) * WPOS + j * 32 + (lane & 31);
+        const int lr = o / WO, wo = o - lr * WO;
+        xbase[j] = ((2 * lt) * NR + 2 * lr) * PITCH + (2 * wo) * 8 + (lane >> 5) * 16;
+    }
+
+    f32x4 pv[3][3];
+    int poff[3];
+    TileAt cur = tile_at(w_begin);
+#pragma unroll
+    for (int u = 0; u < 3; ++u) item_issue(cur, tid + NT * u, 0, 2, 4 * IPP, pv[u], poff[u]);
+
+    auto begin_tile = [&](const TileAt& t, int tid_l) {
+        if (tid_l < BM) {
+            const int m = t.mblk * BM + tid_l;
+            rows[2 * tid_l] = (m < a.M && a.scale) ? a.scale[m] : 1.f;
+            rows[2 * tid_l + 1] = (m < a.M && a.shift) ? a.shift[m] : 0.f;
+        }
+        for (int i = tid_l; i < NPL * NR * 6; i += NT) {
+            const int row = i / 6, e = i - row * 6;
+            *reinterpret_cast<Words2*>(patch + row * PITCH + (e < 2 ? e : 96 + e) * 8) = Words2{0u, 0u};
+        }
+#pragma unroll
+        for (int u = 0; u < 3; ++u) item_commit(pv[u], poff[u]);
+    };
+    begin_tile(cur, tid);
+
+    for (int work = w_begin; work < w_end; ++work) {
+        const int m0 = cur.mblk * BM;
+        int tid_l = tid;
+        asm volatile("" : "+v"(tid_l));
+        const int lane_l = tid_l & 63;
+        const unsigned wvo = (unsigned)(cur.mblk * (BM * STEPS * 64) + lane * 16);
+        bf16x8 aw[WD][2][WM];
+        auto load_w = [&](int s) {
+#pragma unroll
+            for (int kk = 0; kk < 2; ++kk)
+#pragma unroll
+                for (int i = 0; i < WM; ++i)
+                    aw[s % WD][kk][i] = __builtin_bit_cast(bf16x8, __builtin_amdgcn_raw_buffer_load_b128(rw, wvo, ((s * 2 + kk) * WM + i) * 1024, 0));
+        };
+#pragma unroll
+        for (int s = 0; s < WD; ++s) load_w(s);
+        f32x4 sva[3], svb[3];
+        int soffa, soffb;
+        item_issue(cur, tid_l, 1, 2, 4 * IPP, sva, soffa);
+        item_issue(cur, tid_l + NT, 1, 2, 4 * IPP, svb, soffb);
+        __syncthreads();
+
+        f32x16 acc[WM][WN];
+#pragma unroll
+        for (int i = 0; i < WM; ++i)
+#pragma unroll
+            for (int j = 0; j < WN; ++j)
+#pragma unroll
+                for (int r = 0; r < 16; ++r) acc[i][j][r] = 0.f;
+        bf16x8 bv[2][2][WN];
+        auto read_ops = [&](int set, int s) {
+            const int dt = s / 7, dh = s - dt * 7;
+#pragma unroll
+            for (int kk = 0; kk < 2; ++kk)
+#pragma unroll
+                for (int j = 0; j < WN; ++j)
+                    bv[set][kk][j] = *reinterpret_cast<const bf16x8*>(patch + xbase[j] + (dt * NR + dh) * PITCH + kk * 32);
+        };
+        read_ops(0, 0);
+        static_for<0, STEPS>([&](auto step) {
+            constexpr int s = decltype(step)::value;
+            constexpr int set = s & 1;
+            if (s + 1 < STEPS) read_ops(set ^ 1, s + 1);
+            __builtin_amdgcn_sched_barrier(0);
+#pragma unroll
+            for (int kk = 0; kk < 2; ++kk)
+#pragma unroll
+                for (int i = 0; i < WM; ++i)
+#pragma unroll
+                    for (int j = 0; j < WN; ++j)
+                        acc[i][j] = __builtin_amdgcn_mfma_f32_32x32x16_bf16(aw[s % WD][kk][i], bv[set][kk][j], acc[i][j], 0, 0, 0);
+            if (s + WD < STEPS) load_w(s + WD);
+            __builtin_amdgcn_sched_barrier(0);
+            if (s == 1) { item_commit(sva, soffa); item_issue(cur, tid_l + 2 * NT, 1, 2, 4 * IPP, sva, soffa); }
+            if (s == 3) { item_commit(svb, soffb); item_issue(cur, tid_l, 8, 1, 5 * IPP, svb, soffb); }
+            if (s == 5) { item_commit(sva, soffa); item_issue(cur, tid_l + NT, 8, 1, 5 * IPP, sva, soffa); }
+            if (s == 7) { item_commit(svb, soffb); item_issue(cur, tid_l + 2 * NT, 8, 1, 5 * IPP, svb, soffb); }
+            if (s == 9) { item_commit(sva, soffa); item_issue(cur, tid_l + 3 * NT, 8, 1, 5 * IPP, sva, soffa); }
+            if (s == 11) item_commit(svb, soffb);
+            if (s == 13) item_commit(sva, soffa);
+            if (s == 5 || s == 9 || s == 13) __syncthreads();
+        });
+        const TileAt done = cur;
+        auto prefetch_next = [&]() {
+            cur = tile_at(min(work + 1, w_end - 1));
+#pragma unroll
+            for (int u = 0; u < 3; ++u) item_issue(cur, tid_l + NT * u, 0, 2, 4 * IPP, pv[u], poff[u]);
+        };
+        __syncthreads();
+#if !C1T_POOL
+        const int64_t pbase = (int64_t)done.b * a.y_bs + ((int64_t)(done.to0 + lt) * a.Ho + done.ho0) * WO + (wave & 1) * WPOS;
+#endif
+        const bool relu = a.relu != 0;
+#if C1T_POOL
+        {
+#else
+        if (a.half) {
+#endif
+#if !C1T_POOL
+            unsigned short* yh = reinterpret_cast<unsigned short*>(a.out) + pbase;
+#endif
+            unsigned char* tile = patch + wave * (BM * EPI_PITCH);
+            f32x4 ss[WM][4][2];
+#pragma unroll
+            for (int i = 0; i < WM; ++i)
+#pragma unroll
+                for (int q = 0; q < 4; ++q)
+#pragma unroll
+                    for (int u = 0; u < 2; ++u)
+                        ss[i][q][u] = *reinterpret_cast<const f32x4*>(rows + 2 * (i * 32 + 8 * q + 4 * (lane_l >> 5)) + 4 * u);
+#pragma unroll
+            for (int i = 0; i < WM; ++i)
+#pragma unroll
+                for (int q = 0; q < 4; ++q)
+#pragma unroll
+                    for (int rr = 0; rr < 4; ++rr) {
+                        const float sc = ss[i][q][rr >> 1][2 * (rr & 1)], sh = ss[i][q][rr >> 1][2 * (rr & 1) + 1];
+#pragma unroll
+                        for (int j = 0; j < WN; ++j) {
+                            float v = acc[i][j][4 * q + rr] * sc + sh;
+                            if (relu) v = fmaxf(v, 0.f);
+                            *reinterpret_cast<unsigned short*>(tile + (i * 32 + 8 * q + 4 * (lane_l >> 5) + rr) * EPI_PITCH + (j * 32 + (lane_l & 31)) * 2) =
+                                (unsigned short)(cvt_pk_bf16(v, 0.f) & 0xffffu);
+                        }
+                    }
+            __builtin_amdgcn_sched_barrier(0);
+            prefetch_next();
+            __builtin_amdgcn_sched_barrier(0);
+#if C1T_POOL
+            __syncthreads();
+            pool_epilogue(a, po, patch, carry, done, m0, wave, lane_l);
+        }
+#else
+#pragma unroll
+            for (int u = 0; u < BM * 12 / 64; ++u) {
+                const int p = lane_l + 64 * u;
+                const int row = p / 12, c = p - row * 12;
+                if (m0 + row < a.M) {
+                    const Words4 v = *reinterpret_cast<const Words4*>(tile + row * EPI_PITCH + c * 16);
+                    *reinterpret_cast<Words4*>(yh + (int64_t)(m0 + row) * a.y_cs + c * 8) = v;
+                }
+            }
+        } else {
+            float* yf = reinterpret_cast<float*>(a.out) + pbase;
+#pragma unroll
+            for (int i = 0; i < WM; ++i)
+#pragma unroll
+                for (int r = 0; r < 16; ++r) {
+                    const int lr = i * 32 + (r & 3) + 8 * (r >> 2) + 4 * (lane_l >> 5);
+                    const float sc = rows[2 * lr], sh = rows[2 * lr + 1];
+                    if (m0 + lr >= a.M) continue;
+#pragma unroll
+                    for (int j = 0; j < WN; ++j) {
+                        float v = acc[i][j][r] * sc + sh;
+                        if (relu) v = fmaxf(v, 0.f);
+                        yf[(int64_t)(m0 + lr) * a.y_cs + j * 32 + (lane_l & 31)] = v;
+                    }
+                }
+            prefetch_next();
+        }
+#endif
+        __syncthreads();
+        if (work + 1 < w_end) begin_tile(cur, tid_l);
+    }
+}
diff --git a/opental_amd/csrc/conv_select.h b/opental_amd/csrc/conv_select.h
--- a/opental_amd/csrc/conv_select.h
+++ b/opental_amd/csrc/conv_select.h
@@ -126,6 +126,28 @@
 static inline int conv1a_tile_eligible(int To, int Ho) {
     return To % C1T_TT == 0 && Ho % C1T_TR == 0 && !OTAL_OPT("OTAL_CONV_1A_NOTILE");
 }
+struct Conv1aPoolLaunch {
+    int columns, tiles_h;
+    int per_wg, nwg;
+    int plain_per_wg;
+};
+static inline Conv1aPoolLaunch conv1a_pool_launch(int B, int To, int Ho, int M, int wgs) {
+    Conv1aPoolLaunch l;
+    if (wgs < 1) wgs = 1;
+    l.tiles_h = Ho / C1T_TR;
+    l.columns = B * (To / C1T_TT) * ((M + 63) / 64);
+    const int cols_per_wg = (l.columns + wgs - 1) / wgs;
+    l.per_wg = cols_per_wg * l.tiles_h;
+    l.nwg = (l.columns + cols_per_wg - 1) / cols_per_wg;
+    l.plain_per_wg = (l.columns * l.tiles_h + wgs - 1) / wgs;
+    return l;
+}
+static inline int conv1a_pool_taken(int B, int To, int Ho, int M, int wgs) {
+    if (To % C1T_TT || Ho % C1T_TR || B < 1 || M < 1) return 0;
+    const Conv1aPoolLaunch l = conv1a_pool_launch(B, To, Ho, M, wgs);
+    return l.per_wg <= l.plain_per_wg;
+}
+
 static inline bool conv1a_wgrad_eligible(const ConvGeom& g, int prec, const void* x, const void* dy) {
     if (!prec || g.nlev > 1 || OTAL_OPT("OTAL_CONV_NO1AW")) return false;
     if (g.Cin != 3 || g.Cout > 64 || g.kt != 7 || g.kh != 7 || g.kw != 7 || g.st != 2 || g.sh != 2 || g.sw != 2) return false;
diff --git a/opental_amd/csrc/options.h b/opental_amd/csrc/options.h
--- a/opental_amd/csrc/options.h
+++ b/opental_amd/csrc/options.h
@@ -3,6 +3,7 @@
 struct OtalOption { const char* name; int dflt; };
 constexpr OtalOption OTAL_OPTIONS[] = {
     {"OTAL_CONV_1A_NOTILE", 0},           {"OTAL_CONV_1A_WGS", 0},
+    {"OTAL_CONV_1A_POOL", 1},
     {"OTAL_CONV_DIRECT_MINTILES", 140},   {"OTAL_CONV_DIRECT_MINTILES512", 512},
     {"OTAL_CONV_DIRECT_XPF2", 3},         {"OTAL_CONV_NO1A", 0},
     {"OTAL_CONV_NO1AW", 0},               {"OTAL_CONV_NO1DTILE", 0},
```

New measurement: 1015 (median of 6 runs). Within noise of the previous version (+0.8%).
